# mavmap/mavmap

Measured on AMD Instinct MI355X. Metric: global-BA LM iterations/sec, higher is better.
Workload: dtype f64; 1 GPU; C3: 500 images / 200000 points / 2000000 obs global BA, PINHOLE+OPENCV, 2 shared cameras; images=500, points=200000, observations=2000000, parallelism=single GPU, options=max_iter 200, ftol 1e-6, gtol 1e-10, ptol 1e-8, Cauchy a=1, refine intrinsics

## Files before the change

include/mavba.h:

```cpp
#ifndef MAVBA_H_
#define MAVBA_H_

#include <stddef.h>
#include <stdint.h>

#ifdef __cplusplus
extern "C" {
#endif

#define MAVBA_VERSION 1

#define MAVBA_MODEL_PINHOLE 1
#define MAVBA_MODEL_OPENCV 2
#define MAVBA_MODEL_CATA 3
#define MAVBA_MAX_INTR 9

#define MAVBA_CONST_RVEC 1u
#define MAVBA_CONST_TX 2u
#define MAVBA_CONST_TY 4u
#define MAVBA_CONST_TZ 8u
#define MAVBA_CONST_POSE 15u

#define MAVBA_OK 0
#define MAVBA_ERR_INVALID_ARGUMENT (-1)
// ... 135 lines not shown
                        const int64_t* rot_image_ids, const double* rot_rvecs, int64_t n_rot,
                        const mavba_scene_options* scene_options, mavba_problem* problem, const int64_t** image_ids,
                        const int64_t** camera_ids, const int64_t** point_ids);

int mavba_scene_bundle_adjust(mavba_scene* s, const int64_t* free_ids, int64_t n_free, const int64_t* fixed_ids, int64_t n_fixed,
                              const int64_t* fixed_x_ids, int64_t n_fixed_x, const int64_t* gcp_ids, int64_t n_gcp,
                              const int64_t* rot_image_ids, const double* rot_rvecs, int64_t n_rot,
                              const mavba_scene_options* scene_options, const mavba_options* options, mavba_result* result,
                              double* final_cost_px, const int64_t** error_point_ids, const double** error_values,
                              int64_t* num_errors);

typedef struct mavba_session mavba_session;

int mavba_session_create(const mavba_problem* problem,
                         const mavba_options* options, mavba_session** out);
void mavba_session_destroy(mavba_session* s);

int mavba_session_reset(mavba_session* s);

int mavba_session_iterate(mavba_session* s, int32_t max_iters,
                          int32_t* iters_done, int32_t* termination);

int mavba_session_result(mavba_session* s, mavba_result* result);

int mavba_session_get_params(mavba_session* s, double* poses,
                             double* intrinsics, double* points);

int mavba_session_point_errors(mavba_session* s, double* point_error);

int mavba_session_set_params(mavba_session* s, const double* poses, const double* intrinsics, const double* points);

int mavba_session_restart(mavba_session* s);

int mavba_session_filter_points(mavba_session* s, double max_error, const uint8_t* keep, uint8_t* removed,
                                double* errors, int64_t* num_removed);

typedef int (*mavba_allreduce_fn)(void* ctx, void* device_ptr, int64_t count,
                                  int32_t op);
int mavba_session_set_allreduce(mavba_session* s, mavba_allreduce_fn fn,
                                void* ctx, int32_t rank, int32_t world_size);

int mavba_rccl_unique_id(void* out128);
int mavba_session_set_rccl(mavba_session* s, const void* unique_id128, int32_t rank, int32_t world_size);


int mavba_session_eval_jacobian(mavba_session* s, double* cost, double* r,
                                double* Jc, double* Jp, double* Jk);

int mavba_debug_inproc_comms(int32_t world, int32_t calls, int32_t abort_after, int64_t* out);

int mavba_debug_elimination_tree(int32_t num_images, int32_t num_cameras, int64_t npairs, const int32_t* pair_a,
                                 const int32_t* pair_b, int32_t max_depth, int32_t* node_of_image, int32_t* node_parent,
                                 int32_t cap);

int mavba_debug_radix_sort(int32_t n, const uint32_t* keys, int32_t key_bytes, int32_t* order_out, int32_t device);
int64_t mavba_debug_upload_batch(int32_t n, const int64_t* sizes, int64_t arena_bytes, int32_t device);
int mavba_debug_lm_decide(int32_t n, const double* cases, double* out_host, double* out_device, int32_t device);
int mavba_debug_chol_schedule(int32_t nb, int32_t num_nodes, const int32_t* node_begin, const int32_t* node_end, const int32_t* node_parent,
                              int64_t num_pairs, const int32_t* pair_row, const int32_t* pair_col, int32_t cus, double* out,
                              int32_t* tasks_out, int64_t tasks_cap, int64_t* num_tasks, int32_t* upd_out, int64_t upd_cap,
                              int64_t* num_upd, int32_t* chain_info_out);

int mavba_session_reduced_dim(mavba_session* s);
int mavba_session_reduced_system(mavba_session* s, double radius, double* S,
                                 double* v);

int mavba_session_linear_step(mavba_session* s, double radius, double* d_poses,
                              double* d_intr, double* d_points,
                              double* model_cost_change);

int mavba_session_time_jacobian(mavba_session* s, int32_t reps, float* ms_avg);
int mavba_session_set_profiling(mavba_session* s, int32_t on);
int mavba_session_time_front(mavba_session* s, double radius, int32_t reps, float* ms_avg);

typedef struct mavba_session_info {
  int64_t num_obs_kept;
  int32_t reduced_dim;
  int32_t padded_dim;
  int64_t schur_terms[3];
  int64_t schur_blocks;
  int64_t intr_entries;
  int64_t envelope_tiles;
  int64_t dense_tiles;
  double factor_flops;
  double dense_factor_flops;
  int32_t matrix_dim;
  int32_t nd_parts;
  int32_t chain_steps;
  int32_t num_clusters;
  int64_t clustered_points;
  int64_t cluster_partials;
  double cluster_flops;
  double chol_model_forward_us;
  int64_t reduced_store_bytes;
} mavba_session_info;
int mavba_session_get_info(mavba_session* s, mavba_session_info* out);

typedef struct mavba_kernel_stat {
  char name[48];
  int64_t launches;
  double total_ms;
} mavba_kernel_stat;
int mavba_session_kernel_stats(mavba_session* s, mavba_kernel_stat* out,
                               int32_t cap);

int mavba_dense_spd_solve(int32_t n, const double* A, const double* b,
// ... 7 lines not shown
```

mavmap_amd/__init__.py:

```python
from . import _abi
from .problem import BAProblem
from .api import (BundleAdjustmentOptions, MavbaError, Scene, Session, bundle_adjustment,
                  bundle_adjustment_filter_rebundle, pose_refinement, pose_refinement_batch, device_count, dense_spd_solve, rccl_unique_id, load, lib_path, radix_sort_order, elimination_tree, debug_upload_batch)
```

mavmap_amd/api.py:

```python
import ctypes as C
import os
from dataclasses import dataclass

import numpy as np

from . import _abi as A
from .problem import BAProblem

_LIB_PATH = os.path.join(os.path.dirname(os.path.abspath(__file__)), "lib", "libmavba.so")
_lib = None

EXPORTED_SYMBOLS = [
    "mavba_options_init", "mavba_last_error", "mavba_device_count", "mavba_solve", "mavba_pose_refine",
    "mavba_session_create", "mavba_session_destroy", "mavba_session_reset", "mavba_session_iterate",
    "mavba_session_result", "mavba_session_get_params", "mavba_session_point_errors",
    "mavba_session_set_allreduce", "mavba_session_eval_jacobian", "mavba_session_reduced_dim",
    "mavba_session_reduced_system", "mavba_session_linear_step", "mavba_session_time_jacobian", "mavba_session_time_front", "mavba_session_set_profiling",
    "mavba_session_kernel_stats", "mavba_session_get_info", "mavba_dense_spd_solve",
    "mavba_scene_create", "mavba_scene_destroy", "mavba_scene_set_camera", "mavba_scene_set_image", "mavba_scene_add_point2d",
    "mavba_scene_add_points2d", "mavba_scene_set_point3d", "mavba_scene_link", "mavba_scene_delete_point3d", "mavba_scene_get_image", "mavba_scene_get_point3d",
    "mavba_scene_get_camera", "mavba_scene_flatten", "mavba_scene_bundle_adjust",
    "mavba_rccl_unique_id", "mavba_session_set_rccl", "mavba_pose_refine_batch", "mavba_session_set_params", "mavba_session_restart", "mavba_session_filter_points", "mavba_solve_filter_solve",
    "mavba_debug_elimination_tree", "mavba_debug_radix_sort", "mavba_debug_lm_decide", "mavba_debug_chol_schedule",
    "mavba_debug_inproc_comms", "mavba_debug_upload_batch",
]

ALLREDUCE_FN = C.CFUNCTYPE(C.c_int, C.c_void_p, C.c_void_p, C.c_int64, C.c_int32)


class MavbaError(RuntimeError):
    def __init__(self, code, msg):
        super().__init__(f"mavba error {code}: {msg}")
        self.code = code


def lib_path():
    return _LIB_PATH


def load():
    global _lib
    if _lib is not None:
        return _lib
    if not os.path.exists(_LIB_PATH):
        raise MavbaError(A.ERR_NO_DEVICE, f"{_LIB_PATH} is missing: run `python -m mavmap_amd.build` "
                                          "(the HIP extension is mandatory, there is no CPU fallback)")
    L = C.CDLL(_LIB_PATH)
    dp, ip, bp = C.POINTER(C.c_double), C.POINTER(C.c_int32), C.POINTER(C.c_uint8)
    pp, op, rp = C.POINTER(A.CProblem), C.POINTER(A.COptions), C.POINTER(A.CResult)
    sp = C.c_void_p
    L.mavba_options_init.argtypes = [op]
    L.mavba_options_init.restype = None
    L.mavba_last_error.restype = C.c_char_p
    L.mavba_device_count.restype = C.c_int
    L.mavba_solve.argtypes = [pp, op, rp, dp]
    L.mavba_pose_refine.argtypes = [dp, dp, dp, C.c_int32, dp, dp, bp, C.c_int64, op, rp]
    L.mavba_session_create.argtypes = [pp, op, C.POINTER(sp)]
    L.mavba_session_destroy.argtypes = [sp]
    L.mavba_session_destroy.restype = None
    L.mavba_session_reset.argtypes = [sp]
    L.mavba_session_iterate.argtypes = [sp, C.c_int32, ip, ip]
    L.mavba_session_result.argtypes = [sp, rp]
    L.mavba_session_get_params.argtypes = [sp, dp, dp, dp]
    L.mavba_session_point_errors.argtypes = [sp, dp]
    L.mavba_session_set_allreduce.argtypes = [sp, ALLREDUCE_FN, C.c_void_p, C.c_int32, C.c_int32]
    L.mavba_session_eval_jacobian.argtypes = [sp, dp, dp, dp, dp, dp]
    L.mavba_session_reduced_dim.argtypes = [sp]
    L.mavba_session_reduced_system.argtypes = [sp, C.c_double, dp, dp]
    L.mavba_session_linear_step.argtypes = [sp, C.c_double, dp, dp, dp, dp]
    L.mavba_session_time_jacobian.argtypes = [sp, C.c_int32, C.POINTER(C.c_float)]
    L.mavba_session_time_front.argtypes = [sp, C.c_double, C.c_int32, C.POINTER(C.c_float)]
    L.mavba_session_set_profiling.argtypes = [sp, C.c_int32]
    L.mavba_session_kernel_stats.argtypes = [sp, C.POINTER(A.CKernelStat), C.c_int32]
    L.mavba_session_get_info.argtypes = [sp, C.POINTER(A.CSessionInfo)]
    L.mavba_dense_spd_solve.argtypes = [C.c_int32, dp, dp, dp, C.c_int32]
    i64p, i64 = C.POINTER(C.c_int64), C.c_int64
    sop = C.POINTER(A.CSceneOptions)
    L.mavba_scene_create.argtypes = [C.POINTER(sp)]
    L.mavba_scene_destroy.argtypes = [sp]
    L.mavba_scene_destroy.restype = None
    L.mavba_scene_set_camera.argtypes = [sp, i64, C.c_int32, dp]
    L.mavba_scene_set_image.argtypes = [sp, i64, i64, dp, dp]
    L.mavba_scene_add_point2d.argtypes = [sp, i64, i64, dp]
    L.mavba_scene_add_points2d.argtypes = [sp, i64, i64, i64p, dp, i64p]
    L.mavba_scene_set_point3d.argtypes = [sp, i64, dp]
    L.mavba_scene_link.argtypes = [sp, i64, i64]
    L.mavba_scene_delete_point3d.argtypes = [sp, i64]
    L.mavba_scene_get_image.argtypes = [sp, i64, dp, dp]
    L.mavba_scene_get_point3d.argtypes = [sp, i64, dp]
    L.mavba_scene_get_camera.argtypes = [sp, i64, ip, dp]
    lists = [i64p, i64, i64p, i64, i64p, i64, i64p, i64, i64p, dp, i64]
    L.mavba_scene_flatten.argtypes = [sp] + lists + [sop, pp, C.POINTER(i64p), C.POINTER(i64p), C.POINTER(i64p)]
    L.mavba_scene_bundle_adjust.argtypes = [sp] + lists + [sop, op, rp, dp, C.POINTER(i64p), C.POINTER(dp), i64p]
    L.mavba_rccl_unique_id.argtypes = [C.c_void_p]
    L.mavba_session_set_rccl.argtypes = [sp, C.c_void_p, C.c_int32, C.c_int32]
    L.mavba_pose_refine_batch.argtypes = [C.c_int32, C.POINTER(A.CPoseRefineItem), op, rp]
    L.mavba_session_set_params.argtypes = [sp, dp, dp, dp]
    L.mavba_session_restart.argtypes = [sp]
    L.mavba_session_filter_points.argtypes = [sp, C.c_double, bp, bp, dp, C.POINTER(C.c_int64)]
    L.mavba_solve_filter_solve.argtypes = [pp, op, C.c_double, bp, rp, rp, dp, bp, C.POINTER(C.c_int64)]
    L.mavba_debug_elimination_tree.argtypes = [C.c_int32, C.c_int32, C.c_int64, ip, ip, C.c_int32, ip, ip, C.c_int32]
    L.mavba_debug_radix_sort.argtypes = [C.c_int32, C.POINTER(C.c_uint32), C.c_int32, ip, C.c_int32]
    L.mavba_debug_lm_decide.argtypes = [C.c_int32, dp, dp, dp, C.c_int32]
    i32p, i64p = C.POINTER(C.c_int32), C.POINTER(C.c_int64)
    L.mavba_debug_chol_schedule.argtypes = [C.c_int32, C.c_int32, i32p, i32p, i32p, C.c_int64, i32p, i32p, C.c_int32, dp,
                                            i32p, C.c_int64, i64p, i32p, C.c_int64, i64p, i32p]
    for f in EXPORTED_SYMBOLS:
        if f not in ("mavba_options_init", "mavba_last_error", "mavba_session_destroy", "mavba_scene_destroy", "mavba_debug_upload_batch"):
            getattr(L, f).restype = C.c_int
    _lib = L
    return L


def _check(rc):
    if rc != A.OK:
        raise MavbaError(rc, load().mavba_last_error().decode(errors="replace"))


def device_count():
    return int(load().mavba_device_count())


def _d(a):
    return A.ptr(a, C.c_double)


@dataclass
class BundleAdjustmentOptions:
    max_num_iterations: int = 100
    function_tolerance: float = 1e-4
    gradient_tolerance: float = 1e-8
    update_point3D_errors: bool = False
    min_track_len: int = 2
    loss_scale_factor: float = 1.0
    constrain_rotation: bool = False
    constrain_rotation_weight: float = 0.0
    refine_camera_params: bool = False
    print_progress: bool = False
    print_summary: bool = True

    @staticmethod
    def global_ba():
        return BundleAdjustmentOptions(max_num_iterations=200, function_tolerance=1e-6,
                                       gradient_tolerance=1e-10, update_point3D_errors=True,
                                       refine_camera_params=True, print_summary=False)


def make_options(opts=None, **kw):
    o = A.COptions()
    load().mavba_options_init(C.byref(o))
    if isinstance(opts, BundleAdjustmentOptions):
        o.max_num_iterations = int(opts.max_num_iterations)
        o.function_tolerance = float(opts.function_tolerance)
        o.gradient_tolerance = float(opts.gradient_tolerance)
# ... 305 lines not shown

    def reduced_system(self, radius):
        n = load().mavba_session_reduced_dim(self._h)
        S, v = np.zeros((n, n)), np.zeros(n)
        _check(load().mavba_session_reduced_system(self._h, float(radius), _d(S), _d(v)))
        return S, v

    def linear_step(self, radius):
        p = self.problem
        dp, di, dx = np.zeros((p.num_images, 6)), np.zeros((p.num_cameras, 9)), np.zeros((p.num_points, 3))
        mcc = C.c_double()
        _check(load().mavba_session_linear_step(self._h, float(radius), _d(dp), _d(di), _d(dx), C.byref(mcc)))
        return dict(d_poses=dp, d_intr=di, d_points=dx, model_cost_change=mcc.value)

    def set_profiling(self, on):
        _check(load().mavba_session_set_profiling(self._h, 1 if on else 0))

    def time_front(self, radius=1e4, reps=20):
        ms = C.c_float(0)
        _check(load().mavba_session_time_front(self._h, float(radius), int(reps), C.byref(ms)))
        return ms.value

    def time_jacobian(self, reps=20):
        ms = C.c_float()
        _check(load().mavba_session_time_jacobian(self._h, int(reps), C.byref(ms)))
        return float(ms.value)

    def info(self):
        i = A.CSessionInfo()
        _check(load().mavba_session_get_info(self._h, C.byref(i)))
        d = {k: getattr(i, k) for k, _ in i._fields_ if k != "schur_terms"}
        d["schur_terms"] = list(i.schur_terms)
        return d

    def kernel_stats(self):
        buf = (A.CKernelStat * 64)()
        n = load().mavba_session_kernel_stats(self._h, buf, 64)
        return {buf[i].name.decode(): dict(launches=int(buf[i].launches), total_ms=float(buf[i].total_ms))
                for i in range(min(n, 64))}


def elimination_tree(num_images, num_cameras, pairs, max_depth=3):
    pairs = np.ascontiguousarray(pairs, dtype=np.int32).reshape(-1, 2)
    a, b = np.ascontiguousarray(pairs[:, 0]), np.ascontiguousarray(pairs[:, 1])
    node = np.zeros(max(num_images, 1), np.int32)
    parent = np.zeros(4096, np.int32)
    n = load().mavba_debug_elimination_tree(int(num_images), int(num_cameras), len(a), A.ptr(a, C.c_int32), A.ptr(b, C.c_int32),
                                           int(max_depth), A.ptr(node, C.c_int32), A.ptr(parent, C.c_int32), len(parent))
    if n < 0:
        _check(n)
    return node[:num_images], parent[:n]


def radix_sort_order(keys, key_bytes=4, device=-1):
    keys = np.ascontiguousarray(keys, dtype=np.uint32)
    out = np.zeros(len(keys), np.int32)
    _check(load().mavba_debug_radix_sort(len(keys), A.ptr(keys, C.c_uint32), int(key_bytes), A.ptr(out, C.c_int32), device))
    return out


def debug_upload_batch(sizes, arena_bytes=0, device=-1):
    sizes = np.ascontiguousarray(sizes, dtype=np.int64)
    f = load().mavba_debug_upload_batch
    f.restype = C.c_int64
    r = f(C.c_int32(len(sizes)), A.ptr(sizes, C.c_int64), C.c_int64(int(arena_bytes)), C.c_int32(device))
    if r < 0:
        raise MavbaError(A.ERR_HIP, load().mavba_last_error().decode(errors="replace"))
    return int(r)


def debug_lm_decide(cases, device=-1):
    cases = np.ascontiguousarray(cases, dtype=np.float64)
    n = cases.shape[0]
    assert cases.shape[1] == 24
    oh, od = np.zeros((n, 6)), np.zeros((n, 6))
    _check(load().mavba_debug_lm_decide(n, _d(cases), _d(oh), _d(od), device))
    return oh, od


def debug_chol_schedule(nb, nodes, pairs, cus=256):
    nodes = np.ascontiguousarray(nodes, dtype=np.int32).reshape(-1, 3)
    pairs = np.ascontiguousarray(pairs, dtype=np.int32).reshape(-1, 2)
    nbg, ne, npar = (np.ascontiguousarray(nodes[:, k]) for k in range(3))
    pr, pc = np.ascontiguousarray(pairs[:, 0]), np.ascontiguousarray(pairs[:, 1])
    i32 = lambda a: a.ctypes.data_as(C.POINTER(C.c_int32))
    out = np.zeros(8)
    nt, nu = C.c_int64(), C.c_int64()
    ci = np.zeros(nb, np.int32)
    L = load()
    _check(L.mavba_debug_chol_schedule(nb, len(nodes), i32(nbg), i32(ne), i32(npar), len(pairs), i32(pr), i32(pc), cus, _d(out),
                                       None, 0, C.byref(nt), None, 0, C.byref(nu), i32(ci)))
    tasks = np.zeros((max(nt.value, 1), 6), np.int32)
    upd = np.zeros(max(nu.value, 1), np.int32)
    _check(L.mavba_debug_chol_schedule(nb, len(nodes), i32(nbg), i32(ne), i32(npar), len(pairs), i32(pr), i32(pc), cus, _d(out),
                                       i32(tasks), nt.value, C.byref(nt), i32(upd), nu.value, C.byref(nu), i32(ci)))
    tl = [(int(t[0]), int(t[1]), int(t[2]), int(t[3]), [int(x) for x in upd[t[4]:t[5]]]) for t in tasks[:nt.value]]
    return dict(ok=bool(out[0]), model_forward_us=float(out[1]), launch_per_panel_us=float(out[2]), grid=int(out[3]),
                chain_wgs=int(out[4]), tiles=int(out[5]), updates=int(out[6]), nodes=int(out[7]), tasks=tl, chain_info=ci.tolist())


def rccl_unique_id():
    buf = C.create_string_buffer(128)
    _check(load().mavba_rccl_unique_id(buf))
    return buf.raw


# ... 6 lines not shown
```

mavmap_amd/build.py:

```python
import os
import shutil
import subprocess
import sys

ROOT = os.path.dirname(os.path.abspath(__file__))
CSRC = os.path.join(ROOT, "csrc")
LIBDIR = os.path.join(ROOT, "lib")
LIB = os.path.join(LIBDIR, "libmavba.so")
OBJDIR = os.path.join(LIBDIR, "obj")
SOURCES = ["kernels.hip", "schur_rows.hip", "dense_chol.hip", "pose_refine.hip", "host_util.hip", "session_build.hip", "session_lm.hip", "scene.hip", "multi_gpu.hip", "device_setup.hip", "api.hip"]
HEADERS = ["ba_math.h", "dev_reduce.h", "internal.h", "session.h", "lm_decide.h", "lm_bodies.h", "sweep_body.h", os.path.join("..", "..", "include", "mavba.h")]
FLAGS = ["--offload-arch=gfx950", "-O3", "-std=c++17", "-fPIC", "-ffp-contract=on", "-Wall",
         "-Wno-unused-result"]
FILE_FLAGS = {"dense_chol.hip": ["-mllvm", "-amdgpu-mfma-vgpr-form=1"]}


def _hipcc():
    for cand in (shutil.which("hipcc"), "/opt/rocm/bin/hipcc"):
        if cand and os.path.exists(cand):
            return cand
    raise RuntimeError("hipcc not found (ROCm toolchain required to build libmavba.so)")


STAMP = os.path.join(LIBDIR, "build_stamp.json")


def source_digest():
    import hashlib
    h = hashlib.sha256()
    for f in SOURCES + HEADERS:
        with open(os.path.normpath(os.path.join(CSRC, f)), "rb") as fh:
            h.update(f.encode() + b"\0" + fh.read())
    h.update(" ".join(FLAGS).encode())
    h.update(repr(sorted(FILE_FLAGS.items())).encode())
    return h.hexdigest()


def is_current():
    import json
    try:
        return os.path.exists(LIB) and json.load(open(STAMP))["digest"] == source_digest()
    except (OSError, ValueError, KeyError):
        return False


def _stale(target, deps):
    if not os.path.exists(target):
        return True
    t = os.path.getmtime(target)
    return any(os.path.getmtime(d) > t for d in deps if os.path.exists(d))


def build(force=False, verbose=False):
    os.makedirs(OBJDIR, exist_ok=True)
    hdrs = [os.path.normpath(os.path.join(CSRC, h)) for h in HEADERS]
    hipcc = _hipcc()
    objs = []
    for src in SOURCES:
        sp = os.path.join(CSRC, src)
        obj = os.path.join(OBJDIR, src.replace(".hip", ".o"))
        if force or _stale(obj, [sp] + hdrs):
            cmd = [hipcc] + FLAGS + FILE_FLAGS.get(src, []) + ["-c", sp, "-o", obj]
            if verbose:
                print(" ".join(cmd), file=sys.stderr)
            subprocess.check_call(cmd)
        objs.append(obj)
    if force or _stale(LIB, objs):
        cmd = [hipcc, "--offload-arch=gfx950", "-shared", "-fPIC", "-o", LIB] + objs
        if verbose:
            print(" ".join(cmd), file=sys.stderr)
        subprocess.check_call(cmd)
    if not is_current():
        import json
        with open(STAMP, "w") as fh:
            json.dump(dict(digest=source_digest()), fh)
    return LIB


if __name__ == "__main__":
    print(build(force="--force" in sys.argv, verbose=True))
```

mavmap_amd/csrc/api.hip:

```cpp
#include "session.h"
#include "lm_decide.h"

namespace mavba { thread_local std::string g_last_error; }

using namespace mavba;


#define MAVBA_TRY try {
namespace {
struct DeviceGuard {
  int prev = -1;
  explicit DeviceGuard(int dev) {
    if (hipGetDevice(&prev) != hipSuccess) { (void)hipGetLastError(); prev = -1; }
    if (prev != dev) HIP_OK(hipSetDevice(dev)); else prev = -1;
  }
  ~DeviceGuard() { if (prev >= 0) (void)hipSetDevice(prev); }
  DeviceGuard(const DeviceGuard&) = delete;
  DeviceGuard& operator=(const DeviceGuard&) = delete;
};
}
#define MAVBA_SESSION_TRY(s)                                                    \
  try {                                                                         \
    if (!(s)) throw Failure(MAVBA_ERR_INVALID_ARGUMENT, "null session");        \
    DeviceGuard device_guard_((s)->device);
// ... 269 lines not shown
  MAVBA_SESSION_TRY(s)
  s->evaluate();
  if (cost) *cost = s->cost + s->fixed_cost;
  s->ensure_planes();
  launch_jacobian_sweep(s->st, s->sweep_args(s->d_camrec.p, s->d_intr.p, s->d_points.p));
  const size_t S = s->Nstride, N = s->N;
  auto pull = [&](const double* dev, int planes, std::vector<double>& h) {
    h.resize((size_t)planes * S);
    s->download(h.data(), dev, h.size() * 8);
  };
  std::vector<double> hR, hJp, hJc, hJk;
  pull(s->d_R.p, 2, hR); pull(s->d_Jp.p, 6, hJp); pull(s->d_Jc.p, 12, hJc); pull(s->d_Jk.p, 2 * s->KMAX, hJk);
  s->sync();
  s->ensure_perm_host();
  const size_t NO = (size_t)s->NO_all;
  if (r) std::memset(r, 0, NO * 2 * 8);
  if (Jc) std::memset(Jc, 0, NO * 12 * 8);
  if (Jp) std::memset(Jp, 0, NO * 6 * 8);
  if (Jk) std::memset(Jk, 0, NO * 18 * 8);
  for (size_t a = 0; a < N; ++a) {
    const size_t o = (size_t)s->perm[a];
    if (r) for (int e = 0; e < 2; ++e) r[o * 2 + e] = hR[e * S + a];
    if (Jp) for (int e = 0; e < 6; ++e) Jp[o * 6 + e] = hJp[e * S + a];
    if (Jc) for (int e = 0; e < 12; ++e) Jc[o * 12 + e] = hJc[e * S + a];
    if (Jk)
      for (int row = 0; row < 2; ++row)
        for (int k = 0; k < s->KMAX; ++k) Jk[o * 18 + row * 9 + k] = hJk[(size_t)(row * s->KMAX + k) * S + a];
  }
  return MAVBA_OK;
  MAVBA_CATCH
}

int mavba_session_reduced_dim(mavba_session* s) { return s ? s->n_full : 0; }

int mavba_debug_elimination_tree(int32_t NI, int32_t NC, int64_t npairs, const int32_t* pair_a, const int32_t* pair_b, int32_t max_depth,
                                 int32_t* node_of_image, int32_t* node_parent, int32_t cap) {
  MAVBA_TRY
  if (NI < 0 || NC < 0 || npairs < 0 || (npairs > 0 && (!pair_a || !pair_b)) || !node_of_image || !node_parent)
    throw Failure(MAVBA_ERR_INVALID_ARGUMENT, "bad argument");
  std::vector<std::vector<int>> lower(NI);
  for (int64_t k = 0; k < npairs; ++k) {
    const int a = pair_a[k], b = pair_b[k];
    if (a < 0 || a >= NI || b < 0 || b >= NI) throw Failure(MAVBA_ERR_BAD_INDEX, "image pair out of range");
    if (a != b) lower[std::max(a, b)].push_back(std::min(a, b));
  }
  const std::vector<ElimNode> tn = elimination_tree(NI, NC, lower, -1, max_depth);
  if ((int)tn.size() > cap) throw Failure(MAVBA_ERR_INVALID_ARGUMENT, "node_parent too small");
  for (int i = 0; i < NI; ++i) node_of_image[i] = -1;
  for (size_t t = 0; t < tn.size(); ++t) {
    node_parent[t] = tn[t].parent;
    for (int i : tn[t].imgs) node_of_image[i] = (int)t;
  }
  return (int)tn.size();
  MAVBA_CATCH
}

int mavba_session_reduced_system(mavba_session* s, double radius, double* Sout, double* vout) {
  MAVBA_SESSION_TRY(s)
  if (!s->evaluated) s->evaluate();
  s->assemble(radius);
  const int n = s->n_full, m = s->n_mat, nbt = m / 64;
  std::vector<double> store(s->chol_struct.store_doubles());
  s->download(store.data(), s->d_M.p, store.size() * 8);
  s->sync();
  std::vector<double> h((size_t)(m + 1) * m, 0.0);
  const std::vector<int>& slot = s->chol_struct.tile_slot;
  for (int tr = 0; tr <= nbt; ++tr)
    for (int tc = 0; tc < nbt; ++tc) {
      const int sl = slot[(size_t)tr * nbt + tc];
      if (sl < 0) continue;
      const double* T = &store[(size_t)sl << 12];
      const int rows = tr < nbt ? 64 : 1;
      for (int r = 0; r < rows; ++r) std::memcpy(&h[(size_t)(64 * tr + r) * m + 64 * tc], T + 64 * r, 64 * 8);
    }
  std::vector<int> var_col(n, 0);
  for (int t = 0; t < m; ++t) if (s->h_col_var[t] >= 0) var_col[s->h_col_var[t]] = t;
  if (Sout)
    for (int r = 0; r < n; ++r)
      for (int c = 0; c < n; ++c) {
        const int a = std::max(var_col[r], var_col[c]), b = std::min(var_col[r], var_col[c]);
        Sout[(size_t)r * n + c] = h[(size_t)a * m + b];
      }
  if (vout)
    for (int r = 0; r < n; ++r) vout[r] = h[(size_t)m * m + var_col[r]];
  return MAVBA_OK;
  MAVBA_CATCH
}

int mavba_session_linear_step(mavba_session* s, double radius, double* d_poses, double* d_intr, double* d_points,
                              double* model_cost_change) {
  MAVBA_SESSION_TRY(s)
  if (!s->evaluated) s->evaluate();
  double h[SC_COUNT];
  s->linear_step(radius, h);
  if (model_cost_change) *model_cost_change = h[SC_MODEL_CHANGE];
  if (d_poses && s->NI) s->download(d_poses, s->d_delta_cam.p, (size_t)s->NI * 48);
  if (d_intr && s->NC) s->download(d_intr, s->d_delta_cam.p + 6 * (size_t)s->NI, (size_t)s->NC * 72);
  std::vector<double> hdp;
  if (d_points && s->NP) { hdp.resize((size_t)s->NP * 3); s->download(hdp.data(), s->d_delta_pts.p, (size_t)s->NP * 24); }
  s->sync();
  if (d_points) s->to_caller_points(hdp.data(), d_points, 3);
  if (h[SC_FAIL] != 0.0 || h[SC_FAIL_FRONT] != 0.0) throw Failure(MAVBA_ERR_INVALID_ARGUMENT, "linear solve failed (matrix not positive definite)");
  return MAVBA_OK;
  MAVBA_CATCH
}

// ... 417 lines not shown
```

mavmap_amd/csrc/ba_math.h:

```cpp
#ifndef MAVBA_BA_MATH_H_
#define MAVBA_BA_MATH_H_

#include <math.h>

#if defined(__HIPCC__)
#include <hip/hip_runtime.h>
#define MAVBA_HD __host__ __device__ __forceinline__
#else
#define MAVBA_HD inline
#endif

#define MAVBA_M_PINHOLE 1
#define MAVBA_M_OPENCV 2
#define MAVBA_M_CATA 3

namespace mavba {

MAVBA_HD void rot_coeffs(double th2, double& a, double& b, double& c) {
  if (th2 > 1e-6) {
    const double th = sqrt(th2);
    const double s = sin(th), co = cos(th);
    a = s / th;
    b = (1.0 - co) / th2;
    c = (th - s) / (th2 * th);
// ... 167 lines not shown
  double dz0 = 0.0, dz1 = 0.0, dz2 = 1.0;
  if (model == MAVBA_M_CATA) {
    if (nrm > 0.0) {
      const double s = cam[8] / nrm;
      dz0 = s * Xc[0]; dz1 = s * Xc[1]; dz2 = 1.0 + s * Xc[2];
    }
    const double dun = -un * nrm * iz, dvn = -vn * nrm * iz;
    su += (D0 * dun + D1 * dvn) * dk[8];
    sv += (D2 * dun + D3 * dvn) * dk[8];
  }
  const double n0 = iz - un * iz * dz0, n1 = -un * iz * dz1, n2 = -un * iz * dz2;
  const double n3 = -vn * iz * dz0, n4 = iz - vn * iz * dz1, n5 = -vn * iz * dz2;
  A[0] = fx * (D0 * n0 + D1 * n3); A[1] = fx * (D0 * n1 + D1 * n4); A[2] = fx * (D0 * n2 + D1 * n5);
  A[3] = fy * (D2 * n0 + D3 * n3); A[4] = fy * (D2 * n1 + D3 * n4); A[5] = fy * (D2 * n2 + D3 * n5);
  tk0 = ud * dk[0] + dk[2] + fx * su;
  tk1 = vd * dk[1] + dk[3] + fy * sv;
}

MAVBA_HD void obs_residual(int model, const double* rec, const double* cam, const double* X,
                           double uo, double vo, double* r) {
  double Xr[3], Xc[3], u, v;
  transform_point(rec, X, Xr, Xc);
  project<false>(model, cam, Xc, u, v, nullptr, nullptr);
  r[0] = u - uo; r[1] = v - vo;
}

MAVBA_HD void obs_jacobian(int model, const double* rec, const double* cam, const double* X,
                           double uo, double vo, double* r, double* Jc, double* Jp, double* Jk) {
  double Xr[3], Xc[3], u, v, A[6];
  transform_point(rec, X, Xr, Xc);
  project<true>(model, cam, Xc, u, v, A, Jk);
  r[0] = u - uo; r[1] = v - vo;
  const double a = rec[6], b = rec[7], c = rec[8];
#pragma unroll
  for (int i = 0; i < 2; ++i) {
    const double* Ai = &A[3 * i];
    double m1[3], m2[3];
    cross3(Ai, rec, m1);
    cross3(m1, rec, m2);
    Jp[3 * i + 0] = Ai[0] + a * m1[0] + b * m2[0];
    Jp[3 * i + 1] = Ai[1] + a * m1[1] + b * m2[1];
    Jp[3 * i + 2] = Ai[2] + a * m1[2] + b * m2[2];
    double n[3];
    cross3(Ai, Xr, n);
    cross3(n, rec, m1);
    cross3(m1, rec, m2);
    Jc[6 * i + 0] = -(n[0] + b * m1[0] + c * m2[0]);
    Jc[6 * i + 1] = -(n[1] + b * m1[1] + c * m2[1]);
    Jc[6 * i + 2] = -(n[2] + b * m1[2] + c * m2[2]);
    Jc[6 * i + 3] = Ai[0]; Jc[6 * i + 4] = Ai[1]; Jc[6 * i + 5] = Ai[2];
  }
}

MAVBA_HD void obs_backsub_term(int model, const double* rec, const double* cam, const double* X, double uo, double vo,
                               const double* dc, const double* dk, double* r, double* t) {
  double Xr[3], Xc[3], u, v, A[6], tk0, tk1;
  transform_point(rec, X, Xr, Xc);
  project_dk(model, cam, Xc, dk, u, v, A, tk0, tk1);
  r[0] = u - uo; r[1] = v - vo;
  const double a = rec[6], b = rec[7], c = rec[8];
  double m1[3], m2[3], om[3], dX[3];
  cross3(rec, dc, m1);
  cross3(rec, m1, m2);
  om[0] = dc[0] + b * m1[0] + c * m2[0]; om[1] = dc[1] + b * m1[1] + c * m2[1]; om[2] = dc[2] + b * m1[2] + c * m2[2];
  cross3(om, Xr, dX);
  dX[0] += dc[3]; dX[1] += dc[4]; dX[2] += dc[5];
  const double tau0 = A[0] * dX[0] + A[1] * dX[1] + A[2] * dX[2] + tk0;
  const double tau1 = A[3] * dX[0] + A[4] * dX[1] + A[5] * dX[2] + tk1;
  const double q[3] = {A[0] * tau0 + A[3] * tau1, A[1] * tau0 + A[4] * tau1, A[2] * tau0 + A[5] * tau1};
  cross3(rec, q, m1);
  cross3(rec, m1, m2);
  t[0] = q[0] - a * m1[0] + b * m2[0]; t[1] = q[1] - a * m1[1] + b * m2[1]; t[2] = q[2] - a * m1[2] + b * m2[2];
}

MAVBA_HD void cauchy_weight(double s, double b, double inv_b, double& w, double& half_rho) {
  const double sum = 1.0 + s * inv_b;
  half_rho = 0.5 * b * log_obs(sum);
  w = rsqrt_obs(sum);
}

MAVBA_HD void rot_matrix_colmajor(const double* w, double* R) {
  double a, b, c;
  const double th2 = w[0] * w[0] + w[1] * w[1] + w[2] * w[2];
  rot_coeffs(th2, a, b, c);
  const double x = w[0], y = w[1], z = w[2];
  R[0] = 1.0 + b * (x * x - th2); R[3] = -a * z + b * x * y;      R[6] = a * y + b * x * z;
  R[1] = a * z + b * x * y;       R[4] = 1.0 + b * (y * y - th2); R[7] = -a * x + b * y * z;
  R[2] = -a * y + b * x * z;      R[5] = a * x + b * y * z;       R[8] = 1.0 + b * (z * z - th2);
}

MAVBA_HD void rot_prior_eval(const double* w, const double* R0, double weight, double& res,
                             double* jac) {
  const double x = w[0], y = w[1], z = w[2];
  const double th2 = x * x + y * y + z * z;
  double a, b, c;
  rot_coeffs(th2, a, b, c);
  double a1, b1;
  if (th2 > 1e-6) {
    const double th = sqrt(th2), s = sin(th), co = cos(th);
    a1 = (th * co - s) / (th2 * th);
    b1 = (th * s - 2.0 * (1.0 - co)) / (th2 * th2);
  } else {
    a1 = -1.0 / 3.0 + th2 * (1.0 / 30.0 - th2 / 840.0);
    b1 = -1.0 / 12.0 + th2 * (1.0 / 180.0 - th2 / 6720.0);
  }
  const double W[9] = {0, -z, y, z, 0, -x, -y, x, 0};
  const double W2[9] = {x * x - th2, x * y, x * z, x * y, y * y - th2, y * z, x * z, y * z, z * z - th2};
  double R[9];
#pragma unroll
  for (int i = 0; i < 9; ++i) R[i] = ((i % 4 == 0) ? 1.0 : 0.0) + a * W[i] + b * W2[i];
  const int ia[9] = {0, 3, 6, 1, 4, 7, 2, 6, 8};
  double d[9], acc = 0.0;
#pragma unroll
  for (int k = 0; k < 9; ++k) {
    const int cm = ia[k];
    d[k] = R[(cm % 3) * 3 + cm / 3] - R0[k];
    acc += d[k] * d[k];
  }
  const double nrm = sqrt(acc);
  res = weight * nrm;
#pragma unroll
  for (int m = 0; m < 3; ++m) {
    double E[9] = {0, 0, 0, 0, 0, 0, 0, 0, 0};
    if (m == 0) { E[5] = -1; E[7] = 1; }
    if (m == 1) { E[2] = 1; E[6] = -1; }
// ... 55 lines not shown
```

mavmap_amd/csrc/dense_chol.hip:

```cpp
#include "internal.h"
#include "lm_bodies.h"
#include <algorithm>
#include <cstdio>
#include <cstdlib>
#include <iterator>
#include <mutex>
#include <type_traits>

namespace mavba {

namespace {
constexpr int NB = 64;
constexpr int GLD = 66;

typedef double d4 __attribute__((ext_vector_type(4)));

[[maybe_unused]] __device__ __forceinline__ double rsqrt_nr(double d) {
  double y = __builtin_amdgcn_rsq(d);
  const double hd = 0.5 * d;
  y = y * (1.5 - hd * y * y);
  y = y * (1.5 - hd * y * y);
  return y;
}

// ... 99 lines not shown
  const d4 U = __builtin_amdgcn_mfma_f64_16x16x4f64(xa, ba, zero, 0, 0, 0);
  const d4 Xn = __builtin_amdgcn_mfma_f64_16x16x4f64(xa, xacc[B], zero, 0, 0, 0);
  __builtin_amdgcn_sched_barrier(0);
  const double u = li >= c0 + lk ? U[0] : 0.0;
  acc = __builtin_amdgcn_mfma_f64_16x16x4f64(-u, u, acc, 0, 0, 0);
  xacc = __builtin_amdgcn_mfma_f64_16x16x4f64(-u, Xn[0], xacc, 0, 0, 0);
  xfin[B] = Xn[0];
}
__device__ __forceinline__ bool potrf_inv16_b4(d4& acc, d4& xacc, int lane) {
  bool ok = true;
  const int li = lane & 15, lk = lane >> 4;
  d4 xfin = (d4){0.0, 0.0, 0.0, 0.0};
#pragma unroll
  for (int r = 0; r < 4; ++r) xacc[r] = (lk + 4 * r == li) ? 1.0 : 0.0;
  const Pivot4Masks mk = pivot4_masks(lane);
  potrf_inv16_block4<0>(acc, xacc, xfin, lane, ok, mk);
  potrf_inv16_block4<1>(acc, xacc, xfin, lane, ok, mk);
  potrf_inv16_block4<2>(acc, xacc, xfin, lane, ok, mk);
  potrf_inv16_block4<3>(acc, xacc, xfin, lane, ok, mk);
  xacc = xfin;
  const double last = readlane_d(xfin[3], 63);
  return last == last;
}

__device__ __forceinline__ d4 gemm16(const double* A, int lda, const double* B, int ldb, bool transB,
                                     double sign, d4 acc, int lane) {
  const int li = lane & 15, lk = lane >> 4;
#pragma unroll
  for (int kk = 0; kk < 16; kk += 4) {
    const double av = sign * A[li * lda + kk + lk];
    const double bv = transB ? B[li * ldb + kk + lk] : B[(kk + lk) * ldb + li];
    acc = __builtin_amdgcn_mfma_f64_16x16x4f64(av, bv, acc, 0, 0, 0);
  }
  return acc;
}
__device__ __forceinline__ d4 load_d16(const double* C, int ldc, int lane) {
  const int li = lane & 15, lk = lane >> 4;
  d4 v;
#pragma unroll
  for (int r = 0; r < 4; ++r) v[r] = C[(lk + 4 * r) * ldc + li];
  return v;
}
__device__ __forceinline__ void store_d16(double* C, int ldc, d4 v, int lane) {
  const int li = lane & 15, lk = lane >> 4;
#pragma unroll
  for (int r = 0; r < 4; ++r) C[(lk + 4 * r) * ldc + li] = v[r];
}

constexpr bool kPivot4 = true;
constexpr int kFuseBelow = 24;
constexpr int kFuseTasks = 256;
constexpr int kMaxBacksolveGroups = 2048;

__device__ __forceinline__ void wave_lds_sync() {
  __builtin_amdgcn_fence(__ATOMIC_RELEASE, "wavefront");
  __builtin_amdgcn_wave_barrier();
  __builtin_amdgcn_fence(__ATOMIC_ACQUIRE, "wavefront");
}

struct NoPhaseHook { __device__ __forceinline__ void operator()(int) const {} };
struct NoMark { __device__ __forceinline__ void operator()(int) const {} };
struct NoPhase0 { __device__ __forceinline__ void operator()(int) const {} };
template <class Hook = NoPhaseHook, class Mark = NoMark, class Phase0 = NoPhase0>
__device__ __forceinline__ bool tile_potrf_inv_la(double* T, double* Ti, int tid, Hook hook = Hook(), Mark mark = Mark(),
                                                  Phase0 phase0 = Phase0()) {
  const int wv = tid >> 6, lane = tid & 63;
  const d4 zero = (d4){0.0, 0.0, 0.0, 0.0};
  auto Tb = [&](int i, int j) { return T + (16 * i) * GLD + 16 * j; };
  auto Xb = [&](int i, int j) { return Ti + (16 * i) * GLD + 16 * j; };
  auto Lb = [&](int i, int j) { return Ti + (16 * j) * GLD + 16 * i; };
  auto panel = [&](const double* B, const double* Dinv, double* dst) {
    d4 a = gemm16(B, GLD, Dinv, GLD, true, 1.0, zero, lane);
    store_d16(dst, GLD, a, lane);
  };
  auto downdate = [&](double* C, const double* Pa, const double* Pb) {
    d4 a = load_d16(C, GLD, lane);
    a = gemm16(Pa, GLD, Pb, GLD, true, -1.0, a, lane);
    store_d16(C, GLD, a, lane);
  };
  auto chain = [&](double* C, const double* P, int c) -> bool {
    d4 a = load_d16(C, GLD, lane), x;
    if (P) a = gemm16(P, GLD, P, GLD, true, -1.0, a, lane);
    mark(4 * c + 1);
    {
      const int li = lane & 15, lk = lane >> 4;
      bool ident = true;
#pragma unroll
      for (int r = 0; r < 4; ++r) ident = ident && a[r] == ((lk + 4 * r == li) ? 1.0 : 0.0);
      if (__builtin_amdgcn_ballot_w64(!ident) == 0) {
        if (c == 0) phase0(1);
        store_d16(Xb(c, c), GLD, a, lane);
        mark(4 * c + 2);
        return true;
      }
    }
    const bool ok = kPivot4 ? potrf_inv16_b4(a, x, lane) : potrf_inv16(a, x, lane);
    mark(4 * c + 2);
    if (c == 0) phase0(1);
    store_d16(Xb(c, c), GLD, x, lane);
    return ok;
  };
  bool ok = true;
  if (wv == 0) { phase0(0); ok = chain(Tb(0, 0), nullptr, 0); }
  else phase0(2);
  __syncthreads();
  hook(0);
  if (wv != 0) phase0(3);
  if (wv == 0) {
    mark(3);
    panel(Tb(1, 0), Xb(0, 0), Lb(1, 0));
    wave_lds_sync();
// ... 1966 lines not shown
      for (int i = 0; i < NB; i += 2) { s0 = __builtin_fma(Li[i * GLD + lane], in[i], s0); s1 = __builtin_fma(Li[(i + 1) * GLD + lane], in[i + 1], s1); }
      out[lane] = s0 + s1;
    }
  };
  lower_mv(I0, vv, zz);
  if (nb > 1) {
    d4 acc[2][2];
    mfma_quadrant_nt(P, I0, wr, wc, lane, acc);
    load_tile_or_zero(M, sl.s11, W, tid);
    __syncthreads();
    quadrant_to_lds(P, wr, wc, lane, acc);
    __syncthreads();
    d4 upd[2][2], cur[2][2];
    mfma_quadrant_nt(P, P, wr, wc, lane, upd);
    quadrant_from_lds(W, wr, wc, lane, cur);
    quadrant_sub(cur, upd);
    if (wv == 0) {
      double s0 = 0.0, s1 = 0.0;
#pragma unroll 8
      for (int j = 0; j < NB; j += 2) { s0 = __builtin_fma(P[lane * GLD + j], zz[j], s0); s1 = __builtin_fma(P[lane * GLD + j + 1], zz[j + 1], s1); }
      xx[NB + lane] = vv[NB + lane] - (s0 + s1);
    }
    __syncthreads();
    quadrant_to_lds(W, wr, wc, lane, cur);
    __syncthreads();
    ok = tile_factor_inverse(W, I1, tid) && ok;
    __syncthreads();
    lower_mv(I1, xx + NB, zz + NB);
    __syncthreads();
    lower_tmv(I1, zz + NB, xx + NB);
    __syncthreads();
    if (wv == 0) {
      double s0 = 0.0, s1 = 0.0;
#pragma unroll 8
      for (int i = 0; i < NB; i += 2) { s0 = __builtin_fma(P[i * GLD + lane], xx[NB + i], s0); s1 = __builtin_fma(P[(i + 1) * GLD + lane], xx[NB + i + 1], s1); }
      zz[lane] -= s0 + s1;
    }
  }
  __syncthreads();
  lower_tmv(I0, zz, xx);
  __syncthreads();
  if (tid == 0 && !ok) atomicAdd(fail, 1.0);
  for (int c = tid; c < nb_all * NB; c += 256) {
    const double x = c < nb * NB ? xx[c] : 0.0;
    y[c] = x;
    if (scatter) { const int t = scatter[c]; if (t >= 0) y_nat[t] = x; }
  }
  if (UPD) {
    __shared__ double s_red[4];
    __syncthreads();
    const int groups = (U.NI + kUpdImagesPerGroup - 1) / kUpdImagesPerGroup;
    for (int vb = 0; vb < (groups > 0 ? groups : 1); ++vb) {
      update_cameras_body(vb, U.NI, U.NC, U.cam_part, U.radius, U.dmin, U.dmax, y_nat, U.scale_cam, U.img_rec, U.cam_rec, U.poses, U.intr,
                          U.cand_poses, U.cand_intr, U.delta_cam, U.partial3, U.cand_camrec, s_red);
      __syncthreads();
    }
  }
}

static bool chol_small_path() {
  static const bool on = [] { const char* e = std::getenv("MAVBA_CHOL_SMALL"); return !e || std::atoi(e) != 0; }();
  return on;
}
bool dense_spd_solve_is_small(int n_pad, const CholStructure& cs) {
  const int nb = n_pad / NB;
  const int nb_active = cs.active_tiles > 0 ? std::min(cs.active_tiles, nb) : nb;
  return nb_active <= 2 && chol_small_path();
}
bool dense_spd_solve_device(hipStream_t st, double* M, int n_pad, double* y, double* fail,
                            double* diag_ws, double* L, const CholStructure& cs,
                            const int* y_scatter, double* y_nat, bool allow_persistent, hipEvent_t after_factor,
                            const CamUpdateArgs* upd) {
  const int nb = n_pad / NB;
  const int* slot = cs.d_tile_slot;
  double* inv = diag_ws;
  const int nb_active = cs.active_tiles > 0 ? std::min(cs.active_tiles, nb) : nb;
  if (dense_spd_solve_is_small(n_pad, cs)) {
    const bool with_update = upd != nullptr && y_scatter != nullptr && y_nat != nullptr;
    auto hs = [&](int i, int k) { return i <= nb && k < nb ? cs.tile_slot[(size_t)i * nb + k] : -1; };
    const SmallSlots sl{hs(0, 0), nb > 1 ? hs(1, 0) : -1, nb > 1 ? hs(1, 1) : -1, hs(nb, 0), nb > 1 ? hs(nb, 1) : -1};
    if (with_update)
      hipLaunchKernelGGL(k_chol_small<true>, dim3(1), dim3(256), 0, st, M, sl, nb, nb_active, fail, y, y_scatter, y_nat, *upd);
    else
      hipLaunchKernelGGL(k_chol_small<false>, dim3(1), dim3(256), 0, st, M, sl, nb, nb_active, fail, y, y_scatter, y_nat, CamUpdateArgs{});
    if (after_factor) (void)hipEventRecord(after_factor, st);
    return with_update;
  }
  const unsigned epoch = ++cs.epoch;
  if (allow_persistent && cs.persist_ok) {
    CholPersistArgs A;
    A.M = M; A.L = L; A.inv = inv; A.pre = cs.d_pre; A.nb = nb;
    A.tasks = cs.d_tasks; A.wg_begin = cs.d_wg_begin; A.upd = cs.d_upd; A.tile_id = cs.d_tile_id; A.chain_info = cs.d_chain_info;
    A.lflag = cs.d_pflags; A.dflag = cs.d_pflags + cs.persist_tiles; A.pflag = A.dflag + nb; A.abort_flag = A.pflag + 2 * nb;
    A.epoch = epoch; A.fail = fail; A.trace = cs.d_trace;
    static const int drop = [] { const char* e = std::getenv("MAVBA_CHOL_TEST_DROP_WG"); return e ? std::atoi(e) : -1; }();
    A.drop_wg = drop;
    {
      static std::mutex chain_m;
      static hipEvent_t last[64] = {};
      static hipStream_t only_stream[64] = {};
      static bool chained[64] = {};
      int dev = 0;
      (void)hipGetDevice(&dev);
      const bool tracked = dev >= 0 && dev < 64;
      std::lock_guard<std::mutex> g(chain_m);
      if (tracked && !chained[dev]) {
        if (!only_stream[dev]) only_stream[dev] = st;
// ... 63 lines not shown
```

mavmap_amd/csrc/dev_reduce.h:

```cpp
#ifndef MAVBA_DEV_REDUCE_H_
#define MAVBA_DEV_REDUCE_H_
#include <hip/hip_runtime.h>

namespace mavba {

__device__ __forceinline__ double wave_sum(double v) {
#define MAVBA_ROR_ADD(N)                                                                                   \
  {                                                                                                        \
    const int lo = __builtin_amdgcn_update_dpp(0, __double2loint(v), 0x120 | (N), 0xf, 0xf, false);        \
    const int hi = __builtin_amdgcn_update_dpp(0, __double2hiint(v), 0x120 | (N), 0xf, 0xf, false);        \
    v += __hiloint2double(hi, lo);                                                                         \
  }
  MAVBA_ROR_ADD(8) MAVBA_ROR_ADD(4) MAVBA_ROR_ADD(2) MAVBA_ROR_ADD(1)
#undef MAVBA_ROR_ADD
  const int lo = __double2loint(v), hi = __double2hiint(v);
  const double r0 = __hiloint2double(__builtin_amdgcn_readlane(hi, 0), __builtin_amdgcn_readlane(lo, 0));
  const double r1 = __hiloint2double(__builtin_amdgcn_readlane(hi, 16), __builtin_amdgcn_readlane(lo, 16));
  const double r2 = __hiloint2double(__builtin_amdgcn_readlane(hi, 32), __builtin_amdgcn_readlane(lo, 32));
  const double r3 = __hiloint2double(__builtin_amdgcn_readlane(hi, 48), __builtin_amdgcn_readlane(lo, 48));
  return (r0 + r1) + (r2 + r3);
}
__device__ __forceinline__ double wave_max(double v) {
#pragma unroll
  for (int off = 32; off > 0; off >>= 1) v = fmax(v, __shfl_down(v, off, 64));
  return v;
}

__device__ __forceinline__ double dev_rsqrt(double d) {
  const double y = __builtin_amdgcn_rsq(d);
  const double h = __builtin_fma(-(d * y), y, 1.0);
  return __builtin_fma(y * h, __builtin_fma(0.375, h, 0.5), y);
}
__device__ __forceinline__ bool chol3_inv_fast(const double* C, double* Gi) {
  const double r0 = dev_rsqrt(C[0]);
  const double l10 = C[1] * r0, l20 = C[2] * r0;
  const double d1 = __builtin_fma(-l10, l10, C[3]);
  const double r1 = dev_rsqrt(d1);
  const double l21 = __builtin_fma(-l20, l10, C[4]) * r1;
  const double d2 = __builtin_fma(-l21, l21, __builtin_fma(-l20, l20, C[5]));
  const double r2 = dev_rsqrt(d2);
  Gi[0] = r0;
  Gi[1] = -(l10 * r0) * r1;
  Gi[2] = r1;
  Gi[4] = -(l21 * r1) * r2;
  Gi[3] = -__builtin_fma(l21, Gi[1], l20 * r0) * r2;
  Gi[5] = r2;
  return (C[0] > 0.0) && (d1 > 0.0) && (d2 > 0.0);
}

__device__ __forceinline__ double block_sum_256(double v, double* scratch) {
  v = wave_sum(v);
  const int lane = threadIdx.x & 63, wv = threadIdx.x >> 6;
  __syncthreads();
  if (lane == 0) scratch[wv] = v;
  __syncthreads();
  return (scratch[0] + scratch[1]) + (scratch[2] + scratch[3]);
}
// ... 14 lines not shown
```

mavmap_amd/csrc/internal.h:

```cpp
#ifndef MAVBA_INTERNAL_H_
#define MAVBA_INTERNAL_H_

#include <hip/hip_runtime.h>
#include <stdint.h>

#include <utility>
#include <vector>
#include <functional>

namespace mavba {

constexpr int kPoseRec = 24;
constexpr int kIntrRec = 36;

constexpr int kImgRec = 81;
constexpr int kCamRec = 54;
constexpr int kSweepAcc = 135;

struct SweepChunk { int image; int begin; int end; };

enum { BLK_PP = 0, BLK_IP = 1, BLK_II = 2 };

struct SchurBlock {
  int kind;
// ... 155 lines not shown
                      const double* poses, double* res, double* jac, double* cost_partial, const LmSpec& spec = lm_spec_off());

void launch_scales(hipStream_t st, int NI, int NC, int NP, int NPs, int jacobi,
                   const unsigned char* pose_free, const unsigned char* intr_free,
                   const unsigned char* pt_free, const double* img_rec, const double* cam_rec,
                   const double* Cu, double* scale_cam, double* scale_pt);

constexpr int kStateNormsCamBlocks = 64;
void launch_state_norms(hipStream_t st, int NI, int NC, int NP, int NPs, bool cam_part,
                        const unsigned char* pose_free, const unsigned char* intr_free,
                        const unsigned char* pt_free, const double* poses, const double* intr,
                        const double* points, const double* img_rec, const double* cam_rec,
                        const double* gu, double* partial , int* grid_out, const LmSpec& spec = lm_spec_off());


void launch_entries_pose(hipStream_t st, int N, int Nstride, int NPs, const int* obs_img,
                         const int* obs_pt, const unsigned char* pt_free, const double* Jc,
                         const double* Jp, const double* scale_cam, const double* scale_pt,
                         double* Gi, double* h, double* Epose);
void launch_factor_entries_pose(hipStream_t st, int N, int Nstride, int NPs, const int* obs_img, const int* obs_pt,
                                const unsigned char* pt_free, const double* Jc, const double* Jp, const double* scale_cam,
                                const double* scale_pt, double* Gi, double* h, double* Epose, const int* pt_start,
                                const double* Cu, const double* gu, double radius, double dmin, double dmax, double* fail);
void launch_entries_intr(hipStream_t st, int Q, int NI, int NPs, const int* q_pt, const int* q_cam,
                         const double* Wk, const double* scale_cam, const double* scale_pt,
                         const double* Gi, const double* h, double* Eintr);

void launch_schur_chunks(hipStream_t st, int kind, int num_chunks, const SchurChunk* chunks,
                         const int2* terms, const double* Epose, const double* Eintr,
                         double* partial);
int schur_partial_stride(int kind);
void launch_schur_rows(hipStream_t st, const FrontArgs& a, int kmax_intr, bool generic, int num_clusters,
                       const SchurRowsCluster* clusters, const int* tab, const int* cl_lists, const unsigned short* obs_meta,
                       const unsigned long long* lanemap, const unsigned* emit_map, double* part_pp, double* part_ip, double* part_ii,
                       const struct CamSweepArgs* with_sweep = nullptr );
void rows_emit_map(int ni, int nc, int flags, std::vector<unsigned>& pass0, std::vector<unsigned>& pass1);
constexpr unsigned long long kRowsLanesIdentity = 0xFEDCBA9876543210ull;
void launch_schur_clusters(hipStream_t st, ClusterShape shape, int num_clusters, const SchurCluster* clusters, const int* tab,
                           const int* pt_start, const int* q_start, const unsigned short* obs_meta,
                           const unsigned short* q_meta, const unsigned char* pt_clustered, const double* Epose,
                           const double* Eintr, const double* h, int NPs, double* part_pp, double* part_ip,
                           double* part_ii);
void launch_schur_finalize(hipStream_t st, int num_blocks, const SchurBlock* blocks,
                           const double* part_pp, const double* part_ip, const double* part_ii,
                           int NI, int NC, const int* slot, int nb, bool add_base, double radius, double dmin,
                           double dmax, const int* img_cam, const double* img_rec,
                           const double* cam_rec, const double* scale_cam, const int* off_img, const int* off_cam,
                           double* S);
void launch_tiles_copy(hipStream_t st, int num_tiles, const int* tiles, const int* slot, int nb, double* M, double* buf, bool to_buf);
void launch_fix_diag(hipStream_t st, int n_mat, const int* slot, bool add_one, const int* col_var,
                     const double* scale_cam, double* S);

int backsub_points_grid(int NP);
void launch_backsub_points_jvp(hipStream_t st, int NP, int NPs, int NI, double radius, double dmin, double dmax,
                               const SweepArgs& a, const int* pt_start, const double* delta_cam,
                               const unsigned char* pt_free, const double* Gi, const double* h, const double* Cu,
                               const double* gu, const double* scale_pt, double* cand_points, double* delta_points,
                               double* partial , const double* cand_camrec = nullptr, const double* cand_intr = nullptr,
                               double* cost_partial = nullptr);
int update_cameras_groups(int NI);
void launch_update_cameras(hipStream_t st, int NI, int NC, bool cam_part, double radius, double dmin,
                           double dmax, const double* y, const double* scale_cam,
                           const double* img_rec, const double* cam_rec, const double* poses,
                           const double* intr, double* cand_poses, double* cand_intr,
                           double* delta_cam, double* partial3 , double* cand_camrec );

void launch_reduce_cols(hipStream_t st, const double* partial, int rows, int cols, int stride,
                        unsigned max_mask, double* out, bool accumulate);

struct ReduceTask { const double* src; int rows, stride, is_max; const double* src2; int rows2; double* out; };
struct ReduceTasks { ReduceTask t[6]; };
void launch_reduce_tasks(hipStream_t st, const ReduceTasks& tasks, int n, const LmSpec& spec = lm_spec_off());
constexpr int kLmPubDoubles = SC_COUNT + 8;
void launch_lm_snapshot(hipStream_t st, const LmSpec& spec, double* dec, double* host_pub, double seq, double* fail_slots );
void launch_lm_decide_cases(hipStream_t st, int n, const double* in, double* out);
void launch_lm_tail(hipStream_t st, const ReduceTasks& tasks, int n, const LmSpec& spec, double* dec, double* host_pub, double seq, double* fail_slots);
void state_norms_grid(int NI, int NC, int NP, int* gp, int* gc);
struct EvalSmallArgs {
  int NI, NC, NP, NPs, with_cams, cam_part, gp, gc, num_tasks;
  int first_group = 0;
  const int* img_chunk_start; const double* cam_partial; const int* prior_start; const double* prior_res; const double* prior_jac;
  const int* cam_img_start; const int* cam_imgs; double* img_rec; double* cam_rec; double* img_intr_tmp;
  const unsigned char* pose_free; const unsigned char* intr_free; const unsigned char* pt_free;
  const double* poses; const double* intr; const double* points; const double* gu; double* norm_partial;
  ReduceTasks T; LmSpec spec;
  PartialRide ride;
};
void launch_eval_small(hipStream_t st, const EvalSmallArgs& a);
void launch_eval_head_tail(hipStream_t st, const EvalSmallArgs& a);
bool eval_head_tail_fits(int gc);

void launch_points_to_caller(hipStream_t st, int NP, int width, const int* orig, const double* in, double* out);
void launch_point_errors(hipStream_t st, int NP, const int* pt_start, const double* rnorm,
                         const int* pt_count, double* perr);

hipError_t device_alloc(void** p, size_t bytes);
void device_free(void* p);
hipError_t copy_h2d_staged(void* dst, const void* src, size_t bytes, hipStream_t st);
hipError_t copy_d2h_staged_sync(void* dst, const void* src, size_t bytes, hipStream_t st);
void release_staged(hipStream_t st);
bool upload_batch_begin(hipStream_t st);
hipError_t upload_batch_end(bool emit);
hipError_t zero_async(void* p, size_t bytes, hipStream_t st);
void upload_batch_debug_arena(size_t bytes);
int host_threads();
void host_run(int T, const std::function<void(int)>& body);

struct CholFront {
  int k;
  int na;
  int act_off;
  int factor_next;
  int sh_begin;
  long long sh_off;
};
struct CholStep { int kind, front_off, nf, nf0, max_na, merge_begin, init_off, tasks; };
struct CholMerge { int sh_begin; long long sh_off; };
struct CholNode { int begin, end, parent; };
// ... 8 lines not shown
  std::vector<CholMerge> merges;
  std::vector<CholStep> steps;
  std::vector<int> init_tiles;
  int num_leaf_init = 0;
  int chain_steps = 0;
  int num_fronts_max = 0;
  long long envelope_tiles = 0;
  double factor_flops = 0.0;
  size_t shadow_doubles = 0;
  int* d_ints = nullptr;
  int *d_rows = nullptr, *d_seg_of_tile = nullptr, *d_seg_first = nullptr, *d_init = nullptr;
  unsigned* d_flags = nullptr;
  CholFront* d_fronts = nullptr;
  CholMerge* d_merges = nullptr;
  mutable double* d_shadow = nullptr;
  std::vector<int> tile_slot;
  int* d_tile_slot = nullptr;
  long long num_tiles = 0;
  size_t store_doubles() const { return (size_t)std::max<long long>(num_tiles, 1) * 4096; }
  int active_tiles = 0;
  bool persist_ok = false;
  double predicted_forward_us = 0.0;
  int persist_grid = 0;
  int persist_chain_wgs = 0;
  long long persist_tiles = 0;
  long long persist_updates = 0;
  CholTask* d_tasks = nullptr;
  int* d_pints = nullptr;
  int *d_wg_begin = nullptr, *d_upd = nullptr, *d_tile_id = nullptr, *d_chain_info = nullptr;
  unsigned* d_pflags = nullptr;
  double* d_pre = nullptr;
  unsigned long long* d_trace = nullptr;
  std::vector<CholTask> h_tasks;
  std::vector<int> h_wg_begin, h_upd, h_chain_info;
  bool host_only = false;
  int host_only_cus = 256;
  double lpp_estimate_us = 0.0;
  mutable unsigned epoch = 0;
  CholStructure() {}
  CholStructure(const CholStructure&) = delete;
  CholStructure& operator=(const CholStructure&) = delete;
  ~CholStructure();
  void release();
  hipError_t build(int nb, const std::vector<std::pair<int, int>>& tile_pairs, const std::vector<CholNode>& tree,
                   hipStream_t st);
  hipError_t build_dense(int nb);
  hipError_t build_persistent(const std::vector<std::vector<int>>& col_rows, const std::vector<int>& col_step,
                              const std::vector<int>& height, hipStream_t st);
};
struct CamUpdateArgs {
  int NI, NC, cam_part; double radius, dmin, dmax;
  const double* scale_cam; const double* img_rec; const double* cam_rec; const double* poses; const double* intr;
  double* cand_poses; double* cand_intr; double* delta_cam; double* partial3; double* cand_camrec;
};
bool dense_spd_solve_is_small(int n_pad, const CholStructure& cs);
bool dense_spd_solve_device(hipStream_t st, double* M, int n_pad, double* y, double* fail,
                            double* diag_ws, double* L, const CholStructure& cs,
                            const int* y_scatter = nullptr, double* y_nat = nullptr, bool allow_persistent = true,
                            hipEvent_t after_factor = nullptr ,
                            const CamUpdateArgs* upd = nullptr);

}
#endif
```

mavmap_amd/csrc/kernels.hip:

```cpp
#include "internal.h"
#include <cstdlib>
#include <type_traits>
#include "ba_math.h"
#include "dev_reduce.h"
#include "lm_decide.h"
#include "lm_bodies.h"
#include "sweep_body.h"

namespace mavba {

__global__ void k_cam_prepare(int NI, const double* __restrict__ poses, double* __restrict__ camrec) {
  const int i = blockIdx.x * blockDim.x + threadIdx.x;
  if (i >= NI) return;
  double rec[9];
  cam_prepare(poses + 6 * i, rec);
#pragma unroll
  for (int k = 0; k < 9; ++k) camrec[9 * i + k] = rec[k];
}
void launch_cam_prepare(hipStream_t st, int NI, const double* poses, double* camrec) {
  if (NI <= 0) return;
  hipLaunchKernelGGL(k_cam_prepare, dim3((NI + 127) / 128), dim3(128), 0, st, NI, poses, camrec);
}

constexpr int kSweepObsPerBlock = 512;
// ... 1451 lines not shown
        const double g = B.kind == BLK_PP ? img_rec[(size_t)B.row_ent * kImgRec + 21 + r]
                                          : cam_rec[(size_t)B.row_ent * kCamRec + 45 + r];
        base = scale_cam[gr] * g;
      }
      const int C = prow0 + r;
      S[((size_t)slot[nb * nb + (C >> 6)] << 12) + (C & 63)] = base - s;
    }
  };
  for (int idx = lane; idx < PS; idx += 64) apply(idx, strided_sum16(part, PS, idx, B.chunk_begin, B.chunk_end));
}
void launch_schur_finalize(hipStream_t st, int num_blocks, const SchurBlock* blocks,
                           const double* part_pp, const double* part_ip, const double* part_ii,
                           int NI, int NC, const int* slot, int nb, bool add_base, double radius, double dmin,
                           double dmax, const int* img_cam, const double* img_rec,
                           const double* cam_rec, const double* scale_cam, const int* off_img, const int* off_cam,
                           double* S) {
  if (num_blocks <= 0) return;
  hipLaunchKernelGGL(k_schur_finalize, dim3((num_blocks + 3) / 4), dim3(256), 0, st, num_blocks, blocks, part_pp,
                     part_ip, part_ii, NI, NC, slot, nb, add_base ? 1 : 0, radius, dmin, dmax, img_cam, img_rec, cam_rec,
                     scale_cam, off_img, off_cam, S);
}
__global__ void __launch_bounds__(256) k_tiles_copy(int num_tiles, const int* __restrict__ tiles, const int* __restrict__ slot, int nb,
                                                    double* __restrict__ M, double* __restrict__ buf, int to_buf) {
  const int t = blockIdx.x;
  if (t < num_tiles) {
    double2* a = reinterpret_cast<double2*>(M + ((size_t)tiles[t] << 12));
    double2* b = reinterpret_cast<double2*>(buf + ((size_t)t << 12));
    for (int e = threadIdx.x; e < 2048; e += 256) { if (to_buf) b[e] = a[e]; else a[e] = b[e]; }
  } else {
    double* rhs = buf + ((size_t)num_tiles << 12);
    for (int c = (t - num_tiles) * 256 + threadIdx.x; c < nb * 64; c += (gridDim.x - num_tiles) * 256) {
      double* a = M + ((size_t)slot[nb * nb + (c >> 6)] << 12) + (c & 63);
      if (to_buf) rhs[c] = *a; else *a = rhs[c];
    }
  }
}
void launch_tiles_copy(hipStream_t st, int num_tiles, const int* tiles, const int* slot, int nb, double* M, double* buf, bool to_buf) {
  const int extra = std::max(1, std::min(16, (nb * 64 + 1023) / 1024));
  hipLaunchKernelGGL(k_tiles_copy, dim3(num_tiles + extra), dim3(256), 0, st, num_tiles, tiles, slot, nb, M, buf, to_buf ? 1 : 0);
}

__global__ void k_fix_diag(int n_mat, const int* __restrict__ slot, int add_one, const int* __restrict__ col_var,
                           const double* __restrict__ scale_cam, double* __restrict__ S) {
  const int t = blockIdx.x * blockDim.x + threadIdx.x;
  if (t >= n_mat) return;
  const int j = col_var[t];
  if (j < 0 || scale_cam[j] == 0.0) S[((size_t)slot[(t >> 6) * (n_mat >> 6) + (t >> 6)] << 12) + (t & 63) * 65] = add_one ? 1.0 : 0.0;
}
void launch_fix_diag(hipStream_t st, int n_mat, const int* slot, bool add_one, const int* col_var, const double* scale_cam, double* S) {
  hipLaunchKernelGGL(k_fix_diag, dim3((n_mat + 255) / 256), dim3(256), 0, st, n_mat, slot, add_one ? 1 : 0, col_var, scale_cam, S);
}

constexpr int kBsCamsLds = 16;
__global__ void __launch_bounds__(256) k_backsub_points_packed(
    int NP, int NPs, int NI, int NC, int N, int ppb, int nblocks, double radius, double dmin, double dmax, double loss_b, double loss_inv_b,
    const int* __restrict__ pt_start, const int* __restrict__ obs_img, const int* __restrict__ obs_pt,
    const double2* __restrict__ uv, const int* __restrict__ img_cam, const int* __restrict__ cam_model,
    const double* __restrict__ camrec, const double* __restrict__ intr, const double* __restrict__ delta_cam,
    const unsigned char* __restrict__ pt_free, const double* __restrict__ Gi, const double* __restrict__ h,
    const double* __restrict__ Cu, const double* __restrict__ gu, const double* __restrict__ scale_pt,
    const double* __restrict__ points, double* __restrict__ cand_points, double* __restrict__ delta_points,
    double* __restrict__ partial, const double* __restrict__ cand_camrec, const double* __restrict__ cand_intr,
    const unsigned char* __restrict__ pt_active, double* __restrict__ cost_partial) {
  __shared__ double s_t[3][256];
  __shared__ double s_new[3][128];
  __shared__ double s_red[4];
  __shared__ double s_kin[kBsCamsLds][9], s_dk[kBsCamsLds][9];
  __shared__ int s_model[kBsCamsLds];
  const int tid = threadIdx.x;
  const bool cams_lds = NC <= kBsCamsLds;
  double a_step = 0.0, a_model = 0.0, a_x2 = 0.0, a_cost = 0.0;
  const int G = (int)gridDim.x;
  struct Obs { int pt, im; double2 m; };
  auto load_obs = [&](int o) {
    Obs r{0, 0, make_double2(0.0, 0.0)};
    if (N <= 0) return r;
    const int oc = min(o, N - 1);
    r.pt = obs_pt[oc]; r.im = obs_img[oc]; r.m = uv[oc];
    return r;
  };
  auto obs_term = [&](const Obs& q, bool valid, double (&t)[3]) {
    t[0] = t[1] = t[2] = 0.0;
    if (!valid || !pt_free[q.pt]) return;
    const int cam = img_cam[q.im];
    const double X[3] = {points[3 * (size_t)q.pt], points[3 * (size_t)q.pt + 1], points[3 * (size_t)q.pt + 2]};
    double rec[9], kin[9], dc[6], dk[9];
#pragma unroll
    for (int k = 0; k < 9; ++k) rec[k] = camrec[9 * q.im + k];
#pragma unroll
    for (int k = 0; k < 6; ++k) dc[k] = delta_cam[6 * q.im + k];
    int model;
    if (cams_lds) {
      model = s_model[cam];
#pragma unroll
      for (int k = 0; k < 9; ++k) { kin[k] = s_kin[cam][k]; dk[k] = s_dk[cam][k]; }
    } else {
      model = cam_model[cam];
#pragma unroll
      for (int k = 0; k < 9; ++k) { kin[k] = intr[9 * cam + k]; dk[k] = delta_cam[6 * NI + 9 * cam + k]; }
    }
    double r[2], tt[3];
#ifndef MAVBA_BS_SKIP
#define MAVBA_BS_SKIP 0
#endif
    if (MAVBA_BS_SKIP & 1) { r[0] = rec[0] + kin[0] + dc[0] + dk[0]; r[1] = X[0] + q.m.x; tt[0] = rec[3]; tt[1] = X[1]; tt[2] = q.m.y; }
    else
    obs_backsub_term(model, rec, kin, X, q.m.x, q.m.y, dc, dk, r, tt);
    double w, half_rho;
    cauchy_weight(r[0] * r[0] + r[1] * r[1], loss_b, loss_inv_b, w, half_rho);
    const double w2 = w * w;
    t[0] = w2 * tt[0]; t[1] = w2 * tt[1]; t[2] = w2 * tt[2];
  };
  int o0 = 0, o1 = 0, o0n = 0, o1n = 0;
  Obs cur{0, 0, make_double2(0.0, 0.0)};
  if ((int)blockIdx.x < nblocks) {
    const int b0 = (int)blockIdx.x;
    o0 = pt_start[b0 * ppb]; o1 = pt_start[min(b0 * ppb + ppb, NP)];
    if (b0 + G < nblocks) { o0n = pt_start[(b0 + G) * ppb]; o1n = pt_start[min((b0 + G) * ppb + ppb, NP)]; }
    cur = load_obs(o0 + tid);
  }
  if (cams_lds) {
    for (int e = tid; e < 9 * NC; e += 256) { s_kin[e / 9][e % 9] = intr[e]; s_dk[e / 9][e % 9] = delta_cam[6 * NI + e]; }
    for (int c = tid; c < NC; c += 256) s_model[c] = cam_model[c];
    __syncthreads();
  }
  for (int blk = blockIdx.x; blk < nblocks; blk += G) {
    const int p0 = blk * ppb, p1 = min(p0 + ppb, NP);
    const int p = p0 + tid;
    const bool owner = p < p1;
    int o0nn = 0, o1nn = 0;
    Obs nxt = cur;
    if (blk + G < nblocks) {
      nxt = load_obs(o0n + tid);
      if (blk + 2 * G < nblocks) { o0nn = pt_start[(blk + 2 * G) * ppb]; o1nn = pt_start[min((blk + 2 * G) * ppb + ppb, NP)]; }
    }
    int mb = 0, me = 0;
    bool fr = false;
    double G[6] = {0, 0, 0, 0, 0, 0}, sp[3] = {0, 0, 0}, hh[3] = {0, 0, 0}, cu[3] = {0, 0, 0}, gg[3] = {0, 0, 0}, Xo[3] = {0, 0, 0};
    if (owner) {
      mb = pt_start[p]; me = pt_start[p + 1];
      fr = pt_free[p] != 0;
#pragma unroll
      for (int k = 0; k < 3; ++k) Xo[k] = points[3 * (size_t)p + k];
      if (fr) {
        const int dg[3] = {0, 3, 5};
#pragma unroll
        for (int k = 0; k < 6; ++k) G[k] = Gi[k * NPs + p];
#pragma unroll
        for (int k = 0; k < 3; ++k) { sp[k] = scale_pt[k * NPs + p]; hh[k] = h[k * NPs + p]; cu[k] = Cu[dg[k] * NPs + p]; gg[k] = gu[k * NPs + p]; }
      }
    }
    double T[3] = {0.0, 0.0, 0.0};
    for (int base = o0; base < o1; base += 256) {
      const int o = base + tid;
      const Obs q = base == o0 ? cur : load_obs(o);
      double t[3];
      obs_term(q, o < o1, t);
      s_t[0][tid] = t[0]; s_t[1][tid] = t[1]; s_t[2][tid] = t[2];
      __syncthreads();
      if (owner) {
        const int b = max(mb, base), e = (MAVBA_BS_SKIP & 2) ? min(me, max(mb, base) + 1) : min(me, base + 256);
        for (int i = b; i < e; ++i) { T[0] += s_t[0][i - base]; T[1] += s_t[1][i - base]; T[2] += s_t[2][i - base]; }
      }
      __syncthreads();
    }
    if (owner) {
      double d[3] = {0, 0, 0};
      if (fr) {
        const double q0 = -sp[0] * T[0], q1 = -sp[1] * T[1], q2 = -sp[2] * T[2];
        const double z[3] = {q0 * G[0], q0 * G[1] + q1 * G[2], q0 * G[3] + q1 * G[4] + q2 * G[5]};
        const double tt[3] = {hh[0] - z[0], hh[1] - z[1], hh[2] - z[2]};
        double yp[3];
        git_mul(G, tt, yp);
#pragma unroll
        for (int k = 0; k < 3; ++k) {
          const double s = sp[k];
          const double D2 = clampd(s * s * cu[k], dmin, dmax) / radius;
          const double gs = s * gg[k];
          a_model += 0.5 * yp[k] * (gs + D2 * yp[k]);
          d[k] = -yp[k] * s;
          a_step += d[k] * d[k];
        }
      }
#pragma unroll
      for (int k = 0; k < 3; ++k) {
        const double xn = Xo[k] + d[k];
        cand_points[3 * (size_t)p + k] = xn;
        delta_points[3 * (size_t)p + k] = d[k];
        if (fr) a_x2 += xn * xn;
        if (cost_partial) s_new[k][tid] = xn;
      }
    }
    if (cost_partial) {
      __syncthreads();
      for (int base = o0; base < o1; base += 256) {
        const int o = base + tid;
        if (o < o1) {
          const int pt = obs_pt[o], im = obs_img[o];
          const double2 m = uv[o];
          const int cam = img_cam[im];
          double rec[9], kin[9], r[2];
#pragma unroll
          for (int k = 0; k < 9; ++k) rec[k] = cand_camrec[9 * im + k];
#pragma unroll
          for (int k = 0; k < 9; ++k) kin[k] = cand_intr[9 * cam + k];
          const double Xn[3] = {s_new[0][pt - p0], s_new[1][pt - p0], s_new[2][pt - p0]};
          obs_residual(cam_model[cam], rec, kin, Xn, m.x, m.y, r);
          double w, half_rho;
          cauchy_weight(r[0] * r[0] + r[1] * r[1], loss_b, loss_inv_b, w, half_rho);
          if (pt_active && !pt_active[pt]) half_rho = 0.0;
          a_cost += half_rho;
        }
      }
      __syncthreads();
    }
    o0 = o0n; o1 = o1n; o0n = o0nn; o1n = o1nn; cur = nxt;
  }
  const double s0 = block_sum_256(a_step, s_red);
  const double s1 = block_sum_256(a_model, s_red);
  const double s2 = block_sum_256(a_x2, s_red);
  if (threadIdx.x == 0) { partial[3 * blockIdx.x] = s0; partial[3 * blockIdx.x + 1] = s1; partial[3 * blockIdx.x + 2] = s2; }
  if (cost_partial) {
    const double s3 = block_sum_256(a_cost, s_red);
    if (threadIdx.x == 0) cost_partial[blockIdx.x] = s3;
  }
}
int backsub_points_grid(int NP) {
  int gp = (NP + 15) / 16;
  if (gp > 1024) gp = 1024;
  return gp < 1 ? 1 : gp;
}
void launch_backsub_points_jvp(hipStream_t st, int NP, int NPs, int NI, double radius, double dmin, double dmax,
                               const SweepArgs& a, const int* pt_start, const double* delta_cam,
                               const unsigned char* pt_free, const double* Gi, const double* h, const double* Cu,
                               const double* gu, const double* scale_pt, double* cand_points, double* delta_points,
                               double* partial, const double* cand_camrec, const double* cand_intr, double* cost_partial) {
  const int gp = backsub_points_grid(NP);
  const double track = NP > 0 ? (double)a.N / NP : 1.0;
  const int ppb = std::max(1, std::min(128, (int)(224.0 / std::max(track, 1.0))));
  const int nblocks = (NP + ppb - 1) / ppb;
  hipLaunchKernelGGL(k_backsub_points_packed, dim3(gp), dim3(256), 0, st, NP, NPs, NI, a.NC, a.N, ppb, nblocks, radius, dmin, dmax, a.loss_b,
                     a.loss_inv_b, pt_start, a.obs_img, a.obs_pt, a.uv, a.img_cam, a.cam_model, a.camrec, a.intr, delta_cam, pt_free,
                     Gi, h, Cu, gu, scale_pt, a.points, cand_points, delta_points, partial, cand_camrec, cand_intr, a.pt_active,
                     cost_partial);
}

int update_cameras_groups(int NI) { return std::max(1, (NI + kUpdImagesPerGroup - 1) / kUpdImagesPerGroup); }
__global__ void __launch_bounds__(256) k_update_cameras(
    int NI, int NC, int cam_part, double radius, double dmin, double dmax, const double* __restrict__ y,
    const double* __restrict__ scale_cam, const double* __restrict__ img_rec, const double* __restrict__ cam_rec,
    const double* __restrict__ poses, const double* __restrict__ intr, double* cand_poses,
    double* __restrict__ cand_intr, double* __restrict__ delta_cam, double* __restrict__ partial3,
    double* __restrict__ cand_camrec) {
  __shared__ double s_red[4];
  update_cameras_body(blockIdx.x, NI, NC, cam_part, radius, dmin, dmax, y, scale_cam, img_rec, cam_rec, poses, intr, cand_poses, cand_intr,
                      delta_cam, partial3, cand_camrec, s_red);
}
void launch_update_cameras(hipStream_t st, int NI, int NC, bool cam_part, double radius, double dmin,
                           double dmax, const double* y, const double* scale_cam,
                           const double* img_rec, const double* cam_rec, const double* poses,
                           const double* intr, double* cand_poses, double* cand_intr,
                           double* delta_cam, double* partial3, double* cand_camrec) {
  hipLaunchKernelGGL(k_update_cameras, dim3(update_cameras_groups(NI)), dim3(256), 0, st, NI, NC, cam_part ? 1 : 0, radius, dmin,
                     dmax, y, scale_cam, img_rec, cam_rec, poses, intr, cand_poses, cand_intr, delta_cam, partial3, cand_camrec);
}

__global__ void __launch_bounds__(256) k_reduce_cols(const double* __restrict__ partial, int rows, int cols,
                                                     int stride, unsigned max_mask, double* __restrict__ out,
                                                     int accumulate) {
  __shared__ double s_red[4];
  for (int c = 0; c < cols; ++c) {
    const bool mx = (max_mask >> c) & 1u;
    double v = 0.0;
    for (int r = threadIdx.x; r < rows; r += 256) {
      const double x = partial[(size_t)r * stride + c];
      v = mx ? fmax(v, x) : v + x;
    }
    const double t = mx ? block_max_256(v, s_red) : block_sum_256(v, s_red);
    if (threadIdx.x == 0) {
      if (accumulate) out[c] = mx ? fmax(out[c], t) : out[c] + t;
      else out[c] = t;
    }
    __syncthreads();
  }
}
void launch_reduce_cols(hipStream_t st, const double* partial, int rows, int cols, int stride,
                        unsigned max_mask, double* out, bool accumulate) {
  hipLaunchKernelGGL(k_reduce_cols, dim3(1), dim3(256), 0, st, partial, rows, cols, stride, max_mask, out, accumulate ? 1 : 0);
}

__global__ void __launch_bounds__(256) k_reduce_tasks(ReduceTasks T, LmSpec spec) {
  __shared__ double s_red[4];
  if (!lm_spec_go(spec, nullptr)) return;
  reduce_task_body(T.t[blockIdx.x], s_red);
}
__global__ void __launch_bounds__(64) k_lm_snapshot(LmSpec spec, double* dec, double* host_pub, double seq, double* fail_slots) {
  lm_snapshot_body(threadIdx.x, spec, dec, host_pub, seq, fail_slots);
}
__global__ void __launch_bounds__(1024) k_lm_tail(ReduceTasks T, int n, LmSpec spec, double* dec, double* host_pub, double seq, double* fail_slots) {
  __shared__ double s_t[4][2][4];
  reduce_tasks_grouped(T, n, s_t);
  if (threadIdx.x < 64) lm_snapshot_body(threadIdx.x, spec, dec, host_pub, seq, fail_slots);
}
constexpr int kEvalSmallMaxGroups = 40;
__global__ void __launch_bounds__(1024) k_eval_small(EvalSmallArgs a) {
  __shared__ double s_part[16][64];
  __shared__ double s_w[kEvalSmallMaxGroups][2][4];
  __shared__ double s_t[4][2][4];
  if (!lm_spec_go(a.spec, nullptr)) return;
  const int tid = threadIdx.x, g = tid >> 8, lt = tid & 255, wv = (tid >> 6) & 3, lane = tid & 63;
  for (int q = tid; q < a.NI * kSweepAcc; q += 1024)
    camera_reduce_img_elem(q / kSweepAcc, q % kSweepAcc, a.img_chunk_start, a.cam_partial, a.prior_start, a.prior_res, a.prior_jac, a.img_rec,
                           a.img_intr_tmp);
  __syncthreads();
  if (a.with_cams) {
    for (int c = 0; c < a.NC; ++c) {
      if (lane < kCamRec) s_part[tid >> 6][lane] = camera_reduce_cam_part(c, tid >> 6, lane, a.cam_img_start, a.cam_imgs, a.img_intr_tmp);
// ... 146 lines not shown
```

mavmap_amd/csrc/lm_bodies.h:

```cpp
#ifndef MAVBA_LM_BODIES_H_
#define MAVBA_LM_BODIES_H_
#include "internal.h"
#include "ba_math.h"
#include "dev_reduce.h"
#include "lm_decide.h"

namespace mavba {

__device__ __forceinline__ void camera_reduce_img_elem(int i, int e, const int* img_chunk_start, const double* partial,
                                                        const int* prior_start, const double* prior_res, const double* prior_jac,
                                                        double* img_rec, double* img_intr_tmp) {
  const int c0 = img_chunk_start[i], c1 = img_chunk_start[i + 1];
  double s = 0.0;
  int c = c0;
  for (; c + 4 <= c1; c += 4) {
    const double x0 = partial[(size_t)c * kSweepAcc + e], x1 = partial[(size_t)(c + 1) * kSweepAcc + e];
    const double x2 = partial[(size_t)(c + 2) * kSweepAcc + e], x3 = partial[(size_t)(c + 3) * kSweepAcc + e];
    s += x0; s += x1; s += x2; s += x3;
  }
  for (; c < c1; ++c) s += partial[(size_t)c * kSweepAcc + e];
  if (e < 27 && prior_start) {
    for (int q = prior_start[i]; q < prior_start[i + 1]; ++q) {
      const double* j = prior_jac + 3 * q;
      if (e < 21) {
// ... 68 lines not shown
  const double s = block_sum_256(x2, s_red);
  if (threadIdx.x == 0) { partial[2 * vb] = m; partial[2 * vb + 1] = s; }
}

__device__ __forceinline__ double group4_sum(const double* w) { return (w[0] + w[1]) + (w[2] + w[3]); }
__device__ __forceinline__ double group4_max(const double* w) { return fmax(fmax(w[0], w[1]), fmax(w[2], w[3])); }

__device__ __forceinline__ void reduce_task_body(const ReduceTask& t, double* s_red) {
  double v = 0.0;
  for (int r = threadIdx.x; r < t.rows; r += 256) {
    const double x = t.src[(size_t)r * t.stride];
    v = t.is_max ? fmax(v, x) : v + x;
  }
  double total = t.is_max ? block_max_256(v, s_red) : block_sum_256(v, s_red);
  if (t.rows2 > 0) {
    __syncthreads();
    double w = 0.0;
    for (int r = threadIdx.x; r < t.rows2; r += 256) w += t.src2[r];
    total += block_sum_256(w, s_red);
  }
  if (threadIdx.x == 0) *t.out = total;
}

__device__ __forceinline__ void reduce_tasks_grouped(const ReduceTasks& T, int n, double (*s_t)[2][4]) {
  const int tid = threadIdx.x, g = tid >> 8, lt = tid & 255, wv = (tid >> 6) & 3, lane = tid & 63;
  if (g < n) {
    const ReduceTask t = T.t[g];
    double v = 0.0;
    for (int r = lt; r < t.rows; r += 256) {
      const double x = t.src[(size_t)r * t.stride];
      v = t.is_max ? fmax(v, x) : v + x;
    }
    const double red = t.is_max ? wave_max(v) : wave_sum(v);
    double w = 0.0;
    for (int r = lt; r < t.rows2; r += 256) w += t.src2[r];
    const double red2 = wave_sum(w);
    if (lane == 0) { s_t[g][0][wv] = red; s_t[g][1][wv] = red2; }
  }
  __syncthreads();
  if (tid < n) {
    const ReduceTask t = T.t[tid];
    double total = t.is_max ? group4_max(s_t[tid][0]) : group4_sum(s_t[tid][0]);
    if (t.rows2 > 0) total += group4_sum(s_t[tid][1]);
    *t.out = total;
  }
  __syncthreads();
}

constexpr int kUpdImagesPerGroup = 42;
__device__ __forceinline__ void update_cameras_body(int vb, int NI, int NC, int cam_part, double radius, double dmin, double dmax,
                                                    const double* y, const double* scale_cam, const double* img_rec,
                                                    const double* cam_rec, const double* poses, const double* intr,
                                                    double* cand_poses, double* cand_intr, double* delta_cam, double* partial3,
                                                    double* cand_camrec, double* s_red) {
  const int i0 = vb * kUpdImagesPerGroup, i1 = min(i0 + kUpdImagesPerGroup, NI);
  double a_step = 0.0, a_model = 0.0, a_x2 = 0.0;
  auto one = [&](int t) {
    const double s = scale_cam[t];
    double n2, g, x;
    if (t < 6 * NI) {
      const int i = t / 6, e = t % 6;
      n2 = img_rec[(size_t)i * kImgRec + sym_idx(e, e, 6)]; g = img_rec[(size_t)i * kImgRec + 21 + e]; x = poses[t];
    } else {
      const int c = (t - 6 * NI) / 9, k = (t - 6 * NI) % 9;
      n2 = cam_rec[(size_t)c * kCamRec + sym_idx(k, k, 9)]; g = cam_rec[(size_t)c * kCamRec + 45 + k]; x = intr[9 * c + k];
    }
    double d = 0.0;
    if (s != 0.0) {
      const double yy = y[t];
      const double D2 = clampd(s * s * n2, dmin, dmax) / radius;
      d = -yy * s;
      if (cam_part) { a_model += 0.5 * yy * (s * g + D2 * yy); a_step += d * d; }
    }
    const double xn = x + d;
    if (s != 0.0 && cam_part) a_x2 += xn * xn;
    delta_cam[t] = d;
    if (t < 6 * NI) cand_poses[t] = xn; else cand_intr[t - 6 * NI] = xn;
  };
  for (int t = 6 * i0 + threadIdx.x; t < 6 * i1; t += 256) one(t);
  if (vb == 0)
    for (int t = 6 * NI + threadIdx.x; t < 6 * NI + 9 * NC; t += 256) one(t);
  const double s0 = block_sum_256(a_step, s_red);
  const double s1 = block_sum_256(a_model, s_red);
  const double s2 = block_sum_256(a_x2, s_red);
  if (threadIdx.x == 0) { partial3[3 * vb] = s0; partial3[3 * vb + 1] = s1; partial3[3 * vb + 2] = s2; }
  if (cand_camrec) {
    __syncthreads();
    for (int i = i0 + threadIdx.x; i < i1; i += 256) {
      double rec[9];
      cam_prepare(cand_poses + 6 * i, rec);
#pragma unroll
      for (int k = 0; k < 9; ++k) cand_camrec[9 * i + k] = rec[k];
    }
  }
}

__device__ __forceinline__ void lm_snapshot_body(int lane, const LmSpec& spec, double* dec, double* host_pub, double seq, double* fail_slots) {
  const LmDecision d = lm_decide(spec.scal, spec);
  if (lane == 0) { dec[0] = (double)d.code; dec[1] = d.radius; }
  volatile double* out = host_pub;
  double v = 0.0;
  if (lane < SC_COUNT) v = spec.scal[lane];
  else if (lane == SC_COUNT) v = (double)d.code;
  else if (lane == SC_COUNT + 1) v = d.radius;
  else if (lane == SC_COUNT + 2) v = d.decrease_factor;
  else if (lane == SC_COUNT + 3) v = d.rel;
  else if (lane == SC_COUNT + 4) v = d.step_norm;
  else if (lane == SC_COUNT + 5) v = d.cost_change;
  if (lane < SC_COUNT + 6) out[lane] = v;
  __threadfence_system();
  __builtin_amdgcn_wave_barrier();
  if (lane == 0) out[SC_COUNT + 7] = seq;
  if (lane < 2 && fail_slots) fail_slots[lane] = 0.0;
}

}
#endif
```

mavmap_amd/csrc/session.h:

```cpp
#ifndef MAVBA_SESSION_H_
#define MAVBA_SESSION_H_
#include <algorithm>
#include <chrono>
#include <cmath>
#include <cstdio>
#include <cstdlib>
#include <cstring>
#include <condition_variable>
#include <functional>
#include <limits>
#include <map>
#include <memory>
#include <mutex>
#include <shared_mutex>
#include <stdexcept>
#include <string>
#include <thread>
#include <unordered_map>
#include <vector>

#include "../../include/mavba.h"
#include "ba_math.h"
#include "internal.h"

// ... 181 lines not shown
static inline int model_k(int m) { return m == MAVBA_MODEL_PINHOLE ? 4 : m == MAVBA_MODEL_OPENCV ? 8 : 9; }
static inline int round_up(int x, int m) { return (x + m - 1) / m * m; }
static inline double now_s() {
  return std::chrono::duration<double>(std::chrono::steady_clock::now().time_since_epoch()).count();
}

struct KernelTimer { std::string name; long long launches = 0; double total_ms = 0.0; };

template <typename F>
static void parallel_ranges(long long n, F&& body, long long min_parallel = 200000) {
  int T = (int)std::min<long long>(host_threads(), std::max<long long>(n, 1));
  if (n < min_parallel) T = 1;
  if (T == 1) { body(0ll, n); return; }
  host_run(T, [&](int t) { body(n * t / T, n * (t + 1) / T); });
}

}

using namespace mavba;

struct mavba_session {
  mavba_options opt;
  int device = 0;
  hipStream_t st = nullptr;
  int NI = 0, NC = 0, NP = 0, N = 0, Nstride = 32, NPs = 32, KMAX = 4, n_full = 0, n_pad = 64, Q = 0;
  long long NO_all = 0;
  bool any_intr_free = false;
  std::vector<double> h_poses0, h_intr0, h_points0;
  std::vector<int> h_cam_model, h_img_cam, h_pt_start, h_oimg;
  std::vector<long long> perm;
  std::vector<int> h_pt_count_all;
  std::vector<double> h_dropped_rnorm;
  std::vector<double> h_dropped_cost;
  double fixed_cost_priors = 0.0;
  int num_priors_all = 0;
  std::vector<unsigned char> h_pt_removed;
  DevBuf<unsigned char> d_pt_active;
  std::vector<int> h_pt_orig;
  std::vector<unsigned char> h_pose_const, h_intr_const_in, h_pt_const_in;
  std::vector<unsigned char> h_img_used, h_cam_used, h_pt_used;
  std::vector<unsigned char> h_prior_on_img;
  std::vector<unsigned char> h_pose_free, h_intr_free, h_pt_free;
  double fixed_cost = 0.0;
  long long num_residuals = 0, num_residuals_reduced = 0, num_parameters_reduced = 0;
  int num_priors = 0;
  double prior_weight = 0.0;
  double setup_seconds = 0.0, solve_seconds = 0.0;

  DevBuf<double2> d_uv, d_im_uv;
  DevBuf<int> d_obs_img, d_obs_pt, d_pt_start, d_im_pt, d_img_cam, d_cam_model, d_img_chunk_start,
      d_cam_img_start, d_cam_imgs, d_prior_img, d_prior_start, d_q_pt, d_q_cam, d_q_start, d_pt_count;
  DevBuf<FrontTile> d_front_tiles;
  int num_front_tiles = 0;
  DevBuf<FrontTile> d_tail_tiles;
  int num_tail_tiles = 0, tail_begin = 0;
  bool front_ok = false;
  bool fused_ok = false;
  int eval_rows = 0;
  bool front_valid = false;
  double front_radius = 0.0;
  bool fail_slot_clean = false;
  bool planes_ready = false;
  DevBuf<SweepChunk> d_sweep_chunks;
  int num_sweep_chunks = 0;
  DevBuf<unsigned char> d_pose_free, d_intr_free, d_pt_free;
  DevBuf<double> d_prior_R0;
  DevBuf<SchurBlock> d_blocks;
  DevBuf<SchurChunk> d_chunks[3];
  DevBuf<SchurCluster> d_clusters;
  DevBuf<SchurRowsCluster> d_rows_clusters;
  DevBuf<int> d_rows_lists;
  DevBuf<unsigned> d_rows_emit;
  DevBuf<unsigned long long> d_rows_lanes;
  int rows_class_count[kRowsClasses] = {};
  bool rows_ok = false;
  bool rows_generic = false;
  DevBuf<PartialReduce> d_reduce_tasks;
  int num_reduce_tasks = 0;
  DevBuf<int> d_cl_tab, d_cl_lists;
  DevBuf<unsigned short> d_obs_meta, d_q_meta;
  DevBuf<unsigned char> d_pt_clustered;
  int num_clusters = 0, num_slots[3] = {0, 0, 0};
  ClusterShape cl_shape{16, 3};
  long long clustered_points = 0, cluster_partials = 0;
  double cluster_flops = 0.0;
  DevBuf<int2> d_terms[3];
  int num_blocks = 0, num_chunks[3] = {0, 0, 0};
  long long num_terms[3] = {0, 0, 0};
  DevBuf<double> d_poses, d_intr, d_points, d_cposes, d_cintr, d_cpoints, d_poses0, d_intr0, d_points0;
  DevBuf<double> d_camrec, d_ccamrec;
  bool camrec_current = false;
  DevBuf<double> d_R, d_Jp, d_Jc, d_Jk, d_Cu, d_gu, d_Gi, d_h, d_scale_cam, d_scale_pt;
  DevBuf<double> d_sweep_partial, d_camsum , d_img_intr_tmp, d_cam_partial;
  DevBuf<double> d_prior_res, d_prior_jac, d_prior_cost;
  DevBuf<double> d_Epose, d_Eintr, d_Wk, d_part[3];
  DevBuf<double> d_M, d_L, d_y, d_diag_ws, d_delta_cam, d_delta_pts, d_norm_partial, d_step_partial, d_scal;
  DevBuf<double> d_rnorm, d_perr;
  DevBuf<int> d_pt_orig;
  DevBuf<int> d_perm32;
  DevBuf<double> d_pts_out;
  double* d_img_rec = nullptr;
  double* d_cam_rec = nullptr;
  CholStructure chol_struct;
  bool prereduced = false;
  bool sweep_rode_along = false;
  bool setup_batched = false;
  bool M_is_clean = false;
  bool allow_persistent = true;
  bool persist_decided = false;
  bool speculate_on = true;
  void decide_persistent();
  int n_mat = 64, nd_parts = 0;
  std::vector<int> h_off_img, h_off_cam, h_col_var;
  DevBuf<int> d_off, d_col_var;
  DevBuf<double> d_ymat;
  DevBuf<int> d_ar_tiles;
  DevBuf<double> d_ar_buf;
  int num_ar_tiles = 0;

  bool evaluated = false, scales_ready = false, started = false, assembled = false;
  double radius = 1e4, decrease_factor = 2.0;
  double cost = 0.0, x_norm = 0.0, grad_max = 0.0, abs_gtol = 0.0, initial_cost = 0.0;
  int iteration = 0, invalid_steps = 0, n_success = 0, n_fail = 0;
  int termination = MAVBA_TERM_RUNNING;

  mavba_allreduce_fn ar_fn = nullptr;
  void* ar_ctx = nullptr;
  void* rccl_comm = nullptr;
  bool rccl_comm_owned = true;
  std::shared_ptr<RcclGuard> rccl_guard;
  bool sharded() const { return (ar_fn || rccl_comm) && (world > 1 || force_exchange); }
  bool force_exchange = false;
  int rank = 0, world = 1;

  std::vector<KernelTimer> timers;
  struct Pending { int idx; hipEvent_t a, b; bool own_a = true; };
  std::vector<Pending> pending;
  std::vector<hipEvent_t> ev_pool;

  ~mavba_session() {
    if (st) (void)hipStreamSynchronize(st);
    if (rccl_comm && rccl_comm_owned) rccl_comm_destroy(rccl_comm);
    if (lm_pub) lm_pub_free(lm_pub);
    HostSpare<long long>::give(perm); HostSpare<int>::give(h_oimg); HostSpare<double>::give(h_points0);
    for (auto& p : pending) { (void)hipEventDestroy(p.a); (void)hipEventDestroy(p.b); }
    for (auto& e : ev_pool) (void)hipEventDestroy(e);
    if (st) stream_release(st, device);
  }

// ... 47 lines not shown
        rccl_allreduce(rccl_comm, dptr, count, op, st);
      } else {
        rccl_allreduce(rccl_comm, dptr, count, op, st);
      }
      return;
    }
    sync();
    if (ar_fn(ar_ctx, dptr, count, op) != 0) throw Failure(MAVBA_ERR_HIP, "all-reduce hook failed");
  }

  SweepArgs sweep_args(const double* camrec, const double* intr, const double* points) {
    SweepArgs a;
    a.N = N; a.Nstride = Nstride; a.NI = NI; a.NC = NC; a.KMAX = KMAX;
    a.uv = d_uv.p; a.obs_img = d_obs_img.p; a.obs_pt = d_obs_pt.p;
    a.camrec = camrec; a.intr = intr; a.img_cam = d_img_cam.p; a.cam_model = d_cam_model.p;
    a.points = points;
    a.pt_active = h_pt_removed.empty() ? nullptr : d_pt_active.p;
    a.loss_b = opt.loss_scale_factor * opt.loss_scale_factor; a.loss_inv_b = 1.0 / a.loss_b;
    a.R = d_R.p; a.Jp = d_Jp.p; a.Jc = d_Jc.p; a.Jk = d_Jk.p; a.cost_partial = d_sweep_partial.p;
    return a;
  }
  void read_scalars(double* h) {
    HIP_OK(hipMemcpyAsync(h, d_scal.p, SC_COUNT * sizeof(double), hipMemcpyDeviceToHost, st));
    sync();
  }

  void build(const mavba_problem* P, const DeviceRaw* raw = nullptr);
void intr_entries_on_device(const std::vector<unsigned char>& cam_active, std::vector<int>& q_start, std::vector<int>& q_cam);
    void order_on_device(const mavba_problem* P, std::vector<int>& img_start, const DeviceRaw* raw);
  void order_on_host(const mavba_problem* P, const long long* keptp, std::vector<int>& img_start,
                     std::unique_ptr<PinnedBuf<double2>>& uv_h, std::unique_ptr<PinnedBuf<int>>& opt_h,
                     std::unique_ptr<PinnedBuf<double2>>& im_uv_h, std::unique_ptr<PinnedBuf<int>>& im_pt_h);
  void ensure_perm_host();
  void derive_free_flags();
  void finish_structure();
  void choose_elimination_order(const std::vector<SchurBlock>& blocks);
  void reset_state();
  void evaluate(double next_radius = -1.0);
  void evaluate_enqueue(double next_radius = -1.0, const LmSpec& spec = lm_spec_off());
  void launch_front(double r, bool entries, const LmSpec& spec = lm_spec_off(), const CamSweepArgs* with_sweep = nullptr);
  DevBuf<double> d_lm_dec;
  double* lm_pub = nullptr;
  double lm_seq = 0.0;
  LmSpec lm_spec(bool pending_eval) const {
    LmSpec sp{};
    sp.dec = nullptr; sp.scal = d_scal.p;
    sp.radius = radius; sp.decrease_factor = decrease_factor;
    sp.ptol = opt.parameter_tolerance; sp.ftol = opt.function_tolerance; sp.min_rel_dec = opt.min_relative_decrease;
    sp.max_radius = opt.max_trust_region_radius; sp.abs_gtol = abs_gtol; sp.pending_eval = pending_eval ? 1 : 0;
    return sp;
  }
  bool wait_publication(double* h);
  void build_front_tiles(const std::vector<int>& q_start);
  void build_tiles(const std::vector<int>& q_start, int first, DevBuf<FrontTile>& out, int& count);
  void ensure_planes();
  bool fused_now() const { return fused_ok && rows_ok; }
  int eval_cost_rows() const { return front_ok ? eval_rows : (N > 0 ? jacobian_sweep_grid(N) : 0); }
  void take_evaluation(const double* h) { cost = h[SC_COST]; grad_max = h[SC_GRAD_MAX]; x_norm = std::sqrt(h[SC_XNORM2]); }
  void assemble(double r);
  void solve_linear(double r);
  void linear_step(double r, double* h_scal);
  void candidate(double r, double* h_scal);
  void candidate_enqueue(double r, ReduceTasks* tail = nullptr, int* tail_count = nullptr);
  bool merge_small() const;
  bool merge_on = true;
  double pub_wait_seconds = 0.0;
  bool cameras_updated = false;
  double cameras_updated_r = 0.0;
  void start();
  int iterate(int max_iters, int* done);
  void point_errors(double* out);
  void restart();
  long long filter_points(double max_error, const unsigned char* keep, unsigned char* removed_out, double* errors_out);
  void restore_initial_params() {
    HIP_OK(hipMemcpyAsync(d_poses.p, d_poses0.p, (size_t)NI * 6 * 8, hipMemcpyDeviceToDevice, st));
    HIP_OK(hipMemcpyAsync(d_intr.p, d_intr0.p, (size_t)NC * 9 * 8, hipMemcpyDeviceToDevice, st));
    HIP_OK(hipMemcpyAsync(d_points.p, d_points0.p, (size_t)NP * 3 * 8, hipMemcpyDeviceToDevice, st));
    camrec_current = false; evaluated = false; front_valid = false;
  }
  void apply_filter_state();
  void to_caller_points(const double* internal, double* out, int width) const {
    for (int q = 0; q < NP; ++q)
      for (int e = 0; e < width; ++e) out[(size_t)h_pt_orig[q] * width + e] = internal[(size_t)q * width + e];
  }
  void fill_result(mavba_result* r);
};
#endif
```

mavmap_amd/csrc/session_build.hip:

```cpp
#include "session.h"
#include <array>
#include <map>

using namespace mavba;


void mavba_session::derive_free_flags() {
  h_pose_free.assign((size_t)NI * 6, 0);
  h_intr_free.assign((size_t)NC * 9, 0);
  h_pt_free.assign(NP, 0);
  for (int i = 0; i < NI; ++i) {
    if (!h_img_used[i]) continue;
    const unsigned m = h_pose_const[i];
    for (int e = 0; e < 6; ++e) {
      const bool c = e < 3 ? (m & MAVBA_CONST_RVEC) != 0 : (m & (MAVBA_CONST_TX << (e - 3))) != 0;
      h_pose_free[(size_t)i * 6 + e] = c ? 0 : 1;
    }
  }
  any_intr_free = false;
  for (int c = 0; c < NC; ++c) {
    if (!h_cam_used[c] || h_intr_const_in[c]) continue;
    for (int k = 0; k < model_k(h_cam_model[c]); ++k) h_intr_free[(size_t)c * 9 + k] = 1;
    any_intr_free = true;
  }
// ... 333 lines not shown
  img_chunk_start[NI] = (int)sweep_chunks.size();
  num_sweep_chunks = (int)sweep_chunks.size();
  std::vector<int> cam_img_start(NC + 1, 0), cam_imgs(std::max(NI, 1));
  for (int i = 0; i < NI; ++i) cam_img_start[h_img_cam[i] + 1]++;
  for (int c = 0; c < NC; ++c) cam_img_start[c + 1] += cam_img_start[c];
  {
    std::vector<int> cur(cam_img_start.begin(), cam_img_start.end() - 1);
    for (int i = 0; i < NI; ++i) cam_imgs[cur[h_img_cam[i]]++] = i;
  }
  std::vector<int> prior_img(num_priors), prior_start(NI + 1, 0);
  std::vector<double> prior_R0((size_t)num_priors * 9);
  for (int k = 0; k < num_priors; ++k) {
    prior_img[k] = pri[k].first;
    prior_start[pri[k].first + 1]++;
    rot_matrix_colmajor(&P->rot_prior_rvec[3 * pri[k].second], &prior_R0[(size_t)k * 9]);
  }
  for (int i = 0; i < NI; ++i) prior_start[i + 1] += prior_start[i];

  n_full = 6 * NI + 9 * NC;
  n_pad = std::max(64, round_up(n_full, 64));

  lap("image-major view");
  if (!device_order) {
    d_uv.upload_pinned(uv_h->data(), (size_t)N, st); d_obs_img.upload(h_oimg, st); d_obs_pt.upload_pinned(opt_h->data(), (size_t)N, st); d_pt_start.upload(h_pt_start, st);
    d_im_uv.upload_pinned(im_uv_h->data(), (size_t)N, st); d_im_pt.upload_pinned(im_pt_h->data(), (size_t)N, st);
  }
  d_img_cam.upload(h_img_cam, st); d_cam_model.upload(h_cam_model, st);
  d_sweep_chunks.upload(sweep_chunks, st); d_img_chunk_start.upload(img_chunk_start, st);
  d_cam_img_start.upload(cam_img_start, st); d_cam_imgs.upload(cam_imgs, st);
  d_prior_img.upload(prior_img, st); d_prior_start.upload(prior_start, st); d_prior_R0.upload(prior_R0, st);
  d_pt_count.upload(h_pt_count_all, st);
  if (!device_order) { d_pt_orig.upload(h_pt_orig, st); d_points0.upload(h_points0, st); }
  d_pts_out.alloc((size_t)std::max(NP, 1) * 3);
  d_poses0.upload(h_poses0, st); d_intr0.upload(h_intr0, st);
  const size_t nI = std::max(NI, 1), nC = std::max(NC, 1), nP = std::max(NP, 1);
  d_poses.alloc(nI * 6); d_intr.alloc(nC * 9); d_points.alloc(nP * 3);
  d_cposes.alloc(nI * 6); d_cintr.alloc(nC * 9); d_cpoints.alloc(nP * 3);
  d_camrec.alloc(nI * 9); d_ccamrec.alloc(nI * 9);
  d_Cu.alloc((size_t)6 * NPs); d_gu.alloc((size_t)3 * NPs); d_Gi.alloc((size_t)6 * NPs); d_h.alloc((size_t)3 * NPs);
  d_Gi.zero(st); d_h.zero(st);
  d_scale_cam.alloc((size_t)n_pad); d_scale_pt.alloc((size_t)3 * NPs);
  d_scale_cam.zero(st); d_scale_pt.zero(st);
  d_sweep_partial.alloc((size_t)std::max(jacobian_sweep_grid(std::max(N, 1)), kFrontMaxGrid) + 8);
  d_camsum.alloc(nI * kImgRec + nC * kCamRec);
  d_camsum.zero(st);
  d_img_rec = d_camsum.p; d_cam_rec = d_camsum.p + (size_t)NI * kImgRec;
  d_img_intr_tmp.alloc(nI * kCamRec);
  d_cam_partial.alloc((size_t)std::max(num_sweep_chunks, 1) * kSweepAcc);
  d_prior_res.alloc(std::max(num_priors, 1)); d_prior_jac.alloc((size_t)std::max(num_priors, 1) * 3);
  d_prior_cost.alloc(std::max(num_priors, 1));
  d_Epose.alloc((size_t)std::max(N, 1) * kPoseRec);
  d_y.alloc(n_pad); d_y.zero(st);
  d_delta_cam.alloc(n_pad); d_delta_pts.alloc(nP * 3);
  d_norm_partial.alloc((size_t)(512 + kStateNormsCamBlocks) * 2); d_step_partial.alloc((size_t)(1024 + update_cameras_groups(NI) + 2) * 3);
  d_scal.alloc(SC_COUNT); d_scal.zero(st);
  d_rnorm.alloc(std::max(N, 1)); d_perr.alloc(nP);

  lap("alloc + upload");
  derive_free_flags();
  finish_structure();
  lap("finish_structure total");
  setup_batched = false;
  if (batch.open) { batch.open = false; HIP_OK(upload_batch_end(true)); }
  reset_state();
  sync();
  lap("reset + sync");
  setup_seconds = now_s() - t0;
}

namespace mavba {
std::vector<ElimNode> elimination_tree(int NI, int NC, const std::vector<std::vector<int>>& lower, int forced, int max_depth) {
  std::vector<ElimNode> tn;
  typedef ElimNode TNode;
  {
    const int tail = 9 * NC;
    auto tiles_of = [](int cols) { return (cols + 63) / 64; };
    if (forced > 1) {
      std::vector<int> cut(forced);
      for (int q = 0; q < forced; ++q) cut[q] = (int)((long long)q * NI / forced);
      std::vector<std::vector<int>> part(forced);
      std::vector<int> sep;
      int run = 0;
      for (int i = 0; i < NI; ++i) {
        while (run + 1 < forced && i >= cut[run + 1]) ++run;
        int m = i;
        for (int c : lower[i]) m = std::min(m, c);
        if (m < cut[run]) sep.push_back(i); else part[run].push_back(i);
      }
      int np = 0;
      for (auto& pr : part) if (!pr.empty()) { tn.push_back(TNode{std::move(pr), -1}); ++np; }
      if (np >= 2) {
        for (auto& t : tn) t.parent = np;
        tn.push_back(TNode{std::move(sep), -1});
      } else {
        tn.clear();
      }
    } else {
      std::vector<std::vector<int>> adj(NI);
      for (int r = 0; r < NI; ++r)
        for (int c : lower[r]) { adj[r].push_back(c); adj[c].push_back(r); }
      for (auto& a : adj) { std::sort(a.begin(), a.end()); a.erase(std::unique(a.begin(), a.end()), a.end()); }
      bool use_levels = true;
      if (const char* e = std::getenv("MAVBA_ND_LEVELS")) use_levels = std::atoi(e) != 0;
      std::vector<int> pos(NI, -1), level(NI, -1);
      std::function<std::pair<int, int>(std::vector<int>&&, int, int)> rec = [&](std::vector<int>&& M, int depth, int tl) {
        const int n = (int)M.size();
// ... 227 lines not shown
void mavba_session::finish_structure() {
  const bool tt = std::getenv("MAVBA_SETUP_TIMING") != nullptr;
  double tl = now_s();
  auto lap = [&](const char* what) { if (tt) { const double t = now_s(); std::fprintf(stderr, "[setup]   %-26s %8.2f ms\n", what, 1e3 * (t - tl)); tl = t; } };
  d_pose_free.upload(h_pose_free, st); d_intr_free.upload(h_intr_free, st); d_pt_free.upload(h_pt_free, st);
  std::vector<unsigned char> img_active(NI, 0), cam_active(NC, 0);
  for (int i = 0; i < NI; ++i) for (int e = 0; e < 6; ++e) img_active[i] |= h_pose_free[(size_t)i * 6 + e];
  for (int c = 0; c < NC; ++c) for (int k = 0; k < 9; ++k) cam_active[c] |= h_intr_free[(size_t)c * 9 + k];

  std::vector<int> q_start(NP + 1, 0), q_pt, q_cam;
  bool q_on_device = false;
  {
    bool any_cam_active = false;
    for (int c = 0; c < NC; ++c) any_cam_active |= cam_active[c] != 0;
    auto cams_of = [&](int p, int* out) {
      int n = 0;
      for (int a = h_pt_start[p]; a < h_pt_start[p + 1]; ++a) {
        const int c = h_img_cam[h_oimg[a]];
        if (!cam_active[c]) continue;
        int k = 0;
        while (k < n && out[k] != c) ++k;
        if (k == n) out[n++] = c;
      }
      std::sort(out, out + n);
      return n;
    };
    const char* setup_env = std::getenv("MAVBA_SETUP");
    const bool q_host = setup_env && std::string(setup_env) == "host";
    q_on_device = any_cam_active && N >= 50000 && !q_host;
    if (q_on_device) {
      intr_entries_on_device(cam_active, q_start, q_cam);
    } else if (any_cam_active) {
      parallel_ranges(NP, [&](long long p0, long long p1) {
        std::vector<int> tmp(std::max(NC, 1));
        for (long long p = p0; p < p1; ++p) q_start[p + 1] = h_pt_free[p] ? cams_of((int)p, tmp.data()) : 0;
      }, 20000);
      for (int p = 0; p < NP; ++p) q_start[p + 1] += q_start[p];
      q_pt.resize((size_t)q_start[NP]); q_cam.resize((size_t)q_start[NP]);
      parallel_ranges(NP, [&](long long p0, long long p1) {
        std::vector<int> tmp(std::max(NC, 1));
        for (long long p = p0; p < p1; ++p) {
          if (q_start[p + 1] == q_start[p]) continue;
          const int n = cams_of((int)p, tmp.data());
          for (int k = 0; k < n; ++k) { q_pt[(size_t)q_start[p] + k] = (int)p; q_cam[(size_t)q_start[p] + k] = tmp[k]; }
        }
      }, 20000);
    }
  }
  Q = (int)q_cam.size();
  if (!q_on_device) { d_q_start.upload(q_start, st); d_q_pt.upload(q_pt, st); d_q_cam.upload(q_cam, st); }
  d_Eintr.alloc((size_t)std::max(Q, 1) * kIntrRec);
  if (planes_ready) d_Wk.alloc((size_t)std::max(Q, 1) * 27);
  build_front_tiles(q_start);

  lap("flags + intr entries");
  std::vector<unsigned char> pt_mode(NP, 0);
  std::vector<unsigned short> obs_meta((size_t)std::max(N, 1), 0xFFFFu), q_meta((size_t)std::max(Q, 1), 0xFFFFu);
  std::vector<SchurCluster> clusters;
  std::vector<int> cl_imgs, cl_cams;
  {
    cl_shape = ClusterShape{16, 3};
    if (const char* e = std::getenv("MAVBA_CLUSTER_SHAPE")) cl_shape = std::atoi(e) == 12 ? ClusterShape{12, 2} : ClusterShape{16, 3};
  }
  tail_begin = NP;
  while (tail_begin > 0 && (h_pt_start[tail_begin] - h_pt_start[tail_begin - 1] > kTailObs || h_pt_const_in[tail_begin - 1])) --tail_begin;
  const ClusterShape sh = cl_shape;
  const int kClTab = sh.tab(), kClTabPP = sh.tab_pp(), kClTabIP = sh.tab_ip(), kClTabII = sh.tab_ii();
  const int kClImages = sh.images, kClCams = sh.cams;
  std::vector<int> cl_ni, cl_nc, cl_kr;
  auto cam_rows_of = [&](const std::vector<int>& cams) { int k = 0; for (int c : cams) k += model_k(h_cam_model[c]); return k; };
  const bool no_fuse_env = std::getenv("MAVBA_NO_FUSE") != nullptr;
  auto build_clusters = [&](bool rows_mode) {
    clusters.clear(); cl_imgs.clear(); cl_cams.clear(); cl_ni.clear(); cl_nc.clear(); cl_kr.clear();
    std::fill(pt_mode.begin(), pt_mode.end(), 0);
    bool use_clusters = true;
    if (const char* e = std::getenv("MAVBA_CLUSTERS")) use_clusters = std::atoi(e) != 0;
    long long nfree = 0;
    for (int p = 0; p < NP; ++p) nfree += h_pt_free[p] != 0;
    int kMaxPoints = (int)std::min<long long>(256, std::max<long long>(kClBatch, round_up((int)(nfree / 512), kClBatch)));
    if (rows_mode) kMaxPoints = (int)std::min<long long>(kRowsMaxPoints, std::max<long long>(nfree <= 4096 ? kRowsBatch : 2 * kRowsBatch, round_up((int)(nfree / 1024), kRowsBatch)));
    if (const char* e = std::getenv("MAVBA_CLUSTER_POINTS")) kMaxPoints = std::max(1, std::atoi(e));
    if (rows_mode) kMaxPoints = std::min(kMaxPoints, kRowsMaxPoints);
    double kCostF = 20000.0, kCostB[kRowsClasses] = {15400.0, 17500.0, 27500.0};
    if (const char* e = std::getenv("MAVBA_ROWS_COST")) std::sscanf(e, "%lf,%lf,%lf,%lf", &kCostF, &kCostB[0], &kCostB[1], &kCostB[2]);
    const int kRange = 2048;
    const int nranges = (NP + kRange - 1) / kRange;
    std::vector<std::vector<SchurCluster>> r_clusters(nranges);
    std::vector<std::vector<int>> r_imgs(nranges), r_cams(nranges), r_ni(nranges), r_nc(nranges), r_kr(nranges);
    auto do_range = [&](int rg, std::vector<int>& in_cluster, std::vector<int>& in_point) {
      const int r0 = rg * kRange, r_end = std::min(NP, r0 + kRange);
      for (int p = std::max(r0, tail_begin); p < r_end; ++p)
        if (h_pt_free[p] && (h_pt_start[p + 1] > h_pt_start[p] || q_start[p + 1] > q_start[p])) pt_mode[p] = 2;
      const int r1 = std::min(r_end, std::max(r0, tail_begin));
      std::vector<int> cur_i, cur_c, pi;
      int cl_serial = rg * (kRange + 1);
      int cur_p0 = r0, cur_n = 0;
      auto close = [&](int p_end) {
        if (cur_n > 0) {
          r_ni[rg].push_back((int)cur_i.size()); r_nc[rg].push_back((int)cur_c.size()); r_kr[rg].push_back(cam_rows_of(cur_c));
          std::sort(cur_i.begin(), cur_i.end());
          std::sort(cur_c.begin(), cur_c.end());
          r_clusters[rg].push_back(SchurCluster{cur_p0, p_end});
          for (int k = 0; k < kClImages; ++k) r_imgs[rg].push_back(k < (int)cur_i.size() ? cur_i[k] : -1);
          for (int k = 0; k < kClCams; ++k) r_cams[rg].push_back(k < (int)cur_c.size() ? cur_c[k] : -1);
        }
        cur_i.clear(); cur_c.clear(); cur_n = 0; cur_p0 = p_end; ++cl_serial;
// ... 503 lines not shown
      d_rows_clusters.upload(rc, st);
      d_rows_emit.upload(emit_all, st);
      std::vector<int> rl((size_t)std::max(num_clusters, 1) * kRowsLists, -1);
      for (int c = 0; c < num_clusters; ++c) {
        const int o = order[c];
        int* L = &rl[(size_t)c * kRowsLists];
        for (int k = 0; k < kClImages; ++k) { const int img = cl_imgs[(size_t)o * kClImages + k]; L[k] = img; L[kRowsListsCam + k] = img >= 0 ? h_img_cam[img] : -1; }
        for (int k = 0; k < kClCams; ++k) L[kRowsListsCams + k] = cl_cams[(size_t)o * kClCams + k];
      }
      d_rows_lists.upload(rl, st);
      if (std::getenv("MAVBA_CLUSTER_STATS")) {
        long long pts[kRowsClasses] = {}, bat[kRowsClasses] = {};
        for (int c = 0; c < num_clusters; ++c) { const int k = row_class(order[c]); pts[k] += rc[c].p1 - rc[c].p0; bat[k] += (rc[c].p1 - rc[c].p0 + kRowsBatch - 1) / kRowsBatch; }
        for (int k = 0; k < kRowsClasses; ++k)
          std::fprintf(stderr, "[cluster stats] k_schur_rows class %d (%d rows): %d clusters, %lld points, %lld batches\n", k, 16 * kRowsClassNT[k], rows_class_count[k], pts[k], bat[k]);
        long long hist[kClImagesMax + 1][kClCamsMax + 1][2] = {}, unplaced = 0;
        for (int c = 0; c < num_clusters; ++c) { hist[rc[c].ni][rc[c].nc][0]++; hist[rc[c].ni][rc[c].nc][1] += (rc[c].p1 - rc[c].p0 + kRowsBatch - 1) / kRowsBatch; unplaced += (rc[c].flags & kRowsUnplaced) != 0; }
        std::fprintf(stderr, "[cluster stats] k_schur_rows clusters / batches by (images, cameras):");
        for (int i = 0; i <= kClImagesMax; ++i) for (int k = 0; k <= kClCamsMax; ++k) if (hist[i][k][0]) std::fprintf(stderr, " (%d,%d) %lld/%lld", i, k, hist[i][k][0], hist[i][k][1]);
        std::fprintf(stderr, "; clusters that keep the selects: %lld\n", unplaced);
      }
    }
    std::vector<SchurCluster> cl_sorted(clusters.size());
    std::vector<int> tab_sorted(cl_tab.size(), -1);
    std::vector<int> lists_sorted((size_t)std::max(num_clusters, 1) * (kClImages + kClCams), -1);
    for (int c = 0; c < num_clusters; ++c) {
      cl_sorted[c] = clusters[order[c]];
      std::copy(cl_tab.begin() + (size_t)order[c] * kClTab, cl_tab.begin() + (size_t)(order[c] + 1) * kClTab, tab_sorted.begin() + (size_t)c * kClTab);
    }
    for (int c = 0; c < num_clusters; ++c) {
      std::copy(cl_imgs.begin() + (size_t)order[c] * kClImages, cl_imgs.begin() + (size_t)(order[c] + 1) * kClImages, lists_sorted.begin() + (size_t)c * (kClImages + kClCams));
      std::copy(cl_cams.begin() + (size_t)order[c] * kClCams, cl_cams.begin() + (size_t)(order[c] + 1) * kClCams, lists_sorted.begin() + (size_t)c * (kClImages + kClCams) + kClImages);
    }
    d_clusters.upload(cl_sorted, st); d_cl_tab.upload(tab_sorted, st); d_cl_lists.upload(lists_sorted, st);
    d_obs_meta.upload(obs_meta, st); d_q_meta.upload(q_meta, st); d_pt_clustered.upload(ptc, st);
  }
  {
    long long head_observed = 0, head_clustered = 0;
    for (int p = 0; p < tail_begin; ++p) { head_observed += h_pt_start[p + 1] > h_pt_start[p]; head_clustered += pt_mode[p] == 1; }
    const bool no_fuse = std::getenv("MAVBA_NO_FUSE") != nullptr;
    fused_ok = front_ok && !no_fuse && cl_shape.images == 16 && num_clusters > 0 && head_clustered == head_observed &&
               clustered_points == head_clustered && num_clusters <= kFrontMaxGrid;
    num_tail_tiles = 0;
    if (fused_ok && h_pt_start[NP] > h_pt_start[tail_begin]) {
      build_tiles(q_start, tail_begin, d_tail_tiles, num_tail_tiles);
      if ((long long)num_clusters + point_front_grid(num_tail_tiles) > kFrontMaxGrid) { fused_ok = false; num_tail_tiles = 0; }
    }
    rows_ok = rows_ok && fused_ok;
  }
  if (!setup_batched) sync();
  lap("upload terms");
}

void mavba_session::build_front_tiles(const std::vector<int>& q_start) {
  const bool planes_only = std::getenv("MAVBA_FRONT_PLANES") != nullptr;
  front_ok = !planes_only;
  for (int p = 0; p < NP && front_ok; ++p)
    if (q_start[p + 1] - q_start[p] > kFrontQ) front_ok = false;
  num_front_tiles = 0;
  if (front_ok) build_tiles(q_start, 0, d_front_tiles, num_front_tiles);
  else d_front_tiles.upload(std::vector<FrontTile>(), st);
  front_valid = false;
  if (!front_ok) ensure_planes();
}
void mavba_session::build_tiles(const std::vector<int>& q_start, int first, DevBuf<FrontTile>& out, int& count) {
  std::vector<FrontTile> tiles;
  int p0 = first, obs = 0, qs = 0;
  for (int p = first; p < NP; ++p) {
    const int c = h_pt_start[p + 1] - h_pt_start[p], nq = q_start[p + 1] - q_start[p];
    if (p > p0 && (obs + c > kFrontObs || p - p0 >= kFrontPts || qs + nq > kFrontQ)) {
      tiles.push_back(FrontTile{p0, p, h_pt_start[p0], h_pt_start[p], q_start[p0], q_start[p]});
      p0 = p; obs = 0; qs = 0;
    }
    obs += c; qs += nq;
  }
  if (NP > p0) tiles.push_back(FrontTile{p0, NP, h_pt_start[p0], h_pt_start[NP], q_start[p0], q_start[NP]});
  count = (int)tiles.size();
  out.upload(tiles, st);
}

void mavba_session::reset_state() {
  front_valid = false;
  if (!h_pt_removed.empty()) {
    h_pt_removed.clear();
    apply_filter_state();
    M_is_clean = false;
  }
  HIP_OK(hipMemcpyAsync(d_poses.p, d_poses0.p, (size_t)NI * 6 * 8, hipMemcpyDeviceToDevice, st));
  HIP_OK(hipMemcpyAsync(d_intr.p, d_intr0.p, (size_t)NC * 9 * 8, hipMemcpyDeviceToDevice, st));
  HIP_OK(hipMemcpyAsync(d_points.p, d_points0.p, (size_t)NP * 3 * 8, hipMemcpyDeviceToDevice, st));
  evaluated = scales_ready = started = assembled = false;
  camrec_current = false;
  radius = opt.initial_trust_region_radius; decrease_factor = 2.0;
  cost = x_norm = grad_max = abs_gtol = initial_cost = 0.0;
  iteration = invalid_steps = n_success = n_fail = 0;
  termination = MAVBA_TERM_RUNNING;
  solve_seconds = 0.0;
}
```

mavmap_amd/csrc/session_lm.hip:

```cpp
#include "session.h"
#include "lm_decide.h"
#if defined(__x86_64__) || defined(__i386__)
#include <immintrin.h>
#define MAVBA_CPU_RELAX() _mm_pause()
#else
#include <thread>
#define MAVBA_CPU_RELAX() std::this_thread::yield()
#endif

using namespace mavba;


void mavba_session::ensure_planes() {
  if (planes_ready) return;
  d_R.alloc((size_t)2 * Nstride); d_Jp.alloc((size_t)6 * Nstride); d_Jc.alloc((size_t)12 * Nstride);
  d_Jk.alloc((size_t)2 * KMAX * Nstride);
  d_Wk.alloc((size_t)std::max(Q, 1) * 27);
  planes_ready = true;
}

void mavba_session::launch_front(double r, bool entries, const LmSpec& spec, const CamSweepArgs* with_sweep) {
  sweep_rode_along = false;
  prereduced = false;
  FrontArgs f;
// ... 166 lines not shown
                                 d_scale_pt.p, d_Gi.p, d_h.p, d_Epose.p, d_pt_start.p, d_Cu.p, d_gu.p, r, dmin, dmax,
                                 d_scal.p + SC_FAIL);
    });
    timed("entries_intr", [&] {
      launch_entries_intr(st, Q, NI, NPs, d_q_pt.p, d_q_cam.p, d_Wk.p, d_scale_cam.p, d_scale_pt.p, d_Gi.p, d_h.p,
                          d_Eintr.p);
    });
  }
  if (!M_is_clean) {
    timed("memset_S", [&] {
      HIP_OK(hipMemsetAsync(d_M.p, 0, chol_struct.store_doubles() * sizeof(double), st));
      launch_fix_diag(st, n_mat, chol_struct.d_tile_slot, rank == 0, d_col_var.p, d_scale_cam.p, d_M.p);
    });
    M_is_clean = true;
  }
  if (!(front_ok && fused_now())) timed("schur_clusters", [&] {
    launch_schur_clusters(st, cl_shape, num_clusters, d_clusters.p, d_cl_tab.p, d_pt_start.p, d_q_start.p, d_obs_meta.p,
                          d_q_meta.p, d_pt_clustered.p, d_Epose.p, d_Eintr.p, d_h.p, NPs, d_part[0].p, d_part[1].p,
                          d_part[2].p);
  });
  if (num_chunks[0] > 0) timed("schur_chunks_pp", [&] { launch_schur_chunks(st, BLK_PP, num_chunks[0], d_chunks[0].p, d_terms[0].p, d_Epose.p, d_Eintr.p, d_part[0].p); });
  if (num_chunks[1] > 0) timed("schur_chunks_ip", [&] { launch_schur_chunks(st, BLK_IP, num_chunks[1], d_chunks[1].p, d_terms[1].p, d_Epose.p, d_Eintr.p, d_part[1].p); });
  if (num_chunks[2] > 0) timed("schur_chunks_ii", [&] { launch_schur_chunks(st, BLK_II, num_chunks[2], d_chunks[2].p, d_terms[2].p, d_Epose.p, d_Eintr.p, d_part[2].p); });
  const int nbt = n_mat / 64;
  timed("schur_finalize", [&] {
    if (!(prereduced && front_valid && front_radius == r)) launch_partial_reduce(st, num_reduce_tasks, d_reduce_tasks.p, d_part[0].p, d_part[1].p, d_part[2].p);
    launch_schur_finalize(st, num_blocks, d_blocks.p, d_part[0].p, d_part[1].p, d_part[2].p, NI, NC, chol_struct.d_tile_slot, nbt, rank == 0,
                          r, dmin, dmax, d_img_cam.p, d_img_rec, d_cam_rec, d_scale_cam.p, d_off.p, d_off.p + NI, d_M.p);
  });
  if (sharded()) {
    launch_tiles_copy(st, num_ar_tiles, d_ar_tiles.p, chol_struct.d_tile_slot, nbt, d_M.p, d_ar_buf.p, true);
    allreduce(d_ar_buf.p, (long long)num_ar_tiles * 4096 + n_mat, 0);
    launch_tiles_copy(st, num_ar_tiles, d_ar_tiles.p, chol_struct.d_tile_slot, nbt, d_M.p, d_ar_buf.p, false);
  }
  assembled = true;
}

void mavba_session::decide_persistent() {
  if (persist_decided) return;
  if (chol_struct.persist_ok && !sharded()) allow_persistent = persistent_allowed_now();
  persist_decided = true;
}

void mavba_session::solve_linear(double r) {
  decide_persistent();
  assemble(r);
  CamUpdateArgs u;
  const bool with_update = merge_small();
  if (with_update) {
    u.NI = NI; u.NC = NC; u.cam_part = rank == 0 ? 1 : 0; u.radius = r; u.dmin = opt.min_lm_diagonal; u.dmax = opt.max_lm_diagonal;
    u.scale_cam = d_scale_cam.p; u.img_rec = d_img_rec; u.cam_rec = d_cam_rec; u.poses = d_poses.p; u.intr = d_intr.p;
    u.cand_poses = d_cposes.p; u.cand_intr = d_cintr.p; u.delta_cam = d_delta_cam.p;
    u.partial3 = d_step_partial.p + 3 * (size_t)backsub_points_grid(NP); u.cand_camrec = d_ccamrec.p;
  }
  timed_split("chol_factor", "chol_backsolve", [&](hipEvent_t mid) {
    cameras_updated = dense_spd_solve_device(st, d_M.p, n_mat, d_ymat.p, d_scal.p + SC_FAIL, d_diag_ws.p, d_L.p, chol_struct, d_col_var.p, d_y.p,
                                             allow_persistent, mid, with_update ? &u : nullptr);
    cameras_updated_r = r;
  });
  assembled = false;
  fail_slot_clean = false;
  if (!(allow_persistent && chol_struct.persist_ok) || sharded()) M_is_clean = false;
}

void mavba_session::linear_step(double r, double* h) {
  solve_linear(r);
  candidate(r, h);
  if (h[SC_FAIL] >= 1e29 && allow_persistent) {
    std::fprintf(stderr, "mavba: persistent factorisation timed out, falling back to the launch-per-panel schedule\n");
    allow_persistent = false;
    persistent_timed_out();
    solve_linear(r);
    candidate(r, h);
  }
}

void mavba_session::candidate(double r, double* h) {
  candidate_enqueue(r);
  read_scalars(h);
}
void mavba_session::candidate_enqueue(double r, ReduceTasks* tail, int* tail_count) {
  const double dmin = opt.min_lm_diagonal, dmax = opt.max_lm_diagonal;
  const int rows = backsub_points_grid(NP), ugroups = update_cameras_groups(NI);
  if (!(cameras_updated && cameras_updated_r == r))
    timed("update_cameras", [&] {
      launch_update_cameras(st, NI, NC, rank == 0, r, dmin, dmax, d_y.p, d_scale_cam.p, d_img_rec, d_cam_rec,
                            d_poses.p, d_intr.p, d_cposes.p, d_cintr.p, d_delta_cam.p, d_step_partial.p + 3 * (size_t)rows,
                            d_ccamrec.p);
    });
  cameras_updated = false;
  static const long long fuse_max_obs = [] { const char* e = std::getenv("MAVBA_COST_FUSE_MAX_OBS"); return e ? std::atoll(e) : 500000ll; }();
  const bool cost_separate = (long long)N > fuse_max_obs;
  timed("backsub_points", [&] {
    launch_backsub_points_jvp(st, NP, NPs, NI, r, dmin, dmax, sweep_args(d_camrec.p, d_intr.p, d_points.p), d_pt_start.p,
                              d_delta_cam.p, d_pt_free.p, d_Gi.p, d_h.p, d_Cu.p, d_gu.p, d_scale_pt.p, d_cpoints.p,
                              d_delta_pts.p, d_step_partial.p, d_ccamrec.p, d_cintr.p, cost_separate ? nullptr : d_sweep_partial.p);
  });
  SweepArgs a = sweep_args(d_ccamrec.p, d_cintr.p, d_cpoints.p);
  if (cost_separate) timed("cost_only", [&] { launch_cost_only(st, a); });
  if (num_priors > 0)
    timed("rot_prior", [&] {
      launch_rot_prior(st, num_priors, d_prior_img.p, d_prior_R0.p, prior_weight, d_cposes.p, d_prior_res.p,
                       d_prior_jac.p, d_prior_cost.p);
    });
  {
    const int nsweep = N > 0 ? (cost_separate ? jacobian_sweep_grid(N) : rows) : 0;
    ReduceTasks T;
    T.t[0] = ReduceTask{d_step_partial.p, rows + ugroups, 3, 0, nullptr, 0, d_scal.p + SC_STEP_NORM2};
    T.t[1] = ReduceTask{d_step_partial.p + 1, rows + ugroups, 3, 0, nullptr, 0, d_scal.p + SC_MODEL_CHANGE};
    T.t[2] = ReduceTask{d_step_partial.p + 2, rows + ugroups, 3, 0, nullptr, 0, d_scal.p + SC_CAND_XNORM2};
    T.t[3] = ReduceTask{d_sweep_partial.p, nsweep, 1, 0, d_prior_cost.p, num_priors, d_scal.p + SC_NEW_COST};
    if (tail) { *tail = T; *tail_count = 4; }
    else timed("reduce", [&] { launch_reduce_tasks(st, T, 4); });
  }
  if (sharded()) allreduce(d_scal.p + SC_CAND_BEGIN, SC_CAND_COUNT, 0);
}

bool mavba_session::merge_small() const {
  return merge_on && !sharded() && NI <= 64 && NC <= 8 && NP <= 8192 && dense_spd_solve_is_small(n_mat, chol_struct);
}

void mavba_session::start() {
  { const char* e = std::getenv("MAVBA_MERGE"); merge_on = !e || std::atoi(e) != 0; }
  { const char* e = std::getenv("MAVBA_SPECULATE"); speculate_on = !e || std::atoi(e) != 0; }
  decide_persistent();
  evaluate();
  initial_cost = cost + fixed_cost;
  const double g0 = std::max(grad_max, std::numeric_limits<double>::epsilon());
  abs_gtol = opt.gradient_tolerance * g0;
  started = true;
  if (num_residuals_reduced == 0 || num_parameters_reduced == 0) { termination = MAVBA_TERM_FUNCTION_TOLERANCE; return; }
  if (grad_max <= abs_gtol) { termination = MAVBA_TERM_GRADIENT_TOLERANCE; return; }
  if (opt.print_progress) {
    std::printf("%4s %14s %12s %10s %10s %10s %10s\n", "iter", "cost", "cost_change", "|gradient|", "|step|", "tr_ratio", "tr_radius");
    std::printf("%4d %14.6e %12.2e %10.2e %10.2e %10.2e %10.2e\n", 0, cost + fixed_cost, 0.0, grad_max, 0.0, 0.0, radius);
  }
}

bool mavba_session::wait_publication(double* h) {
  volatile double* pub = lm_pub;
  const double t_end = now_s() + 2.0;
  for (long long spin = 0;; ++spin) {
    if (pub[SC_COUNT + 7] == lm_seq) break;
    MAVBA_CPU_RELAX();
    if ((spin & 0xFFFF) == 0xFFFF && now_s() > t_end) return false;
  }
  std::atomic_thread_fence(std::memory_order_acquire);
  for (int i = 0; i < SC_COUNT; ++i) h[i] = pub[i];
// ... 234 lines not shown
```

Before: 1302 iter/s.

## Tile back-substitution by point observation counts and precompute per-image step records

Points are grouped on the host into tiles of at most 64 observations or 64 points. The back-substitution kernel is rewritten to work per wavefront over these tiles, with a separate path for long tiles, prefetched gathers and a launch-bounds occupancy hint. The camera update kernel now writes a per-image rotated step record once, so each observation no longer recomputes the cross products from the camera delta. The default observation limit for fusing the cost into back-substitution is raised, so this 2M-observation problem now takes the fused path. In exchange the change adds a tile table, a new per-image buffer, more kernel complexity, and a build hook that rebuilds and adjusts the timestamp of an oracle reference shim.

Result: no change. 1303 iter/s (median of 3 runs) (+0.1%).

```diff
diff --git a/include/mavba.h b/include/mavba.h
--- a/include/mavba.h
+++ b/include/mavba.h
@@ -211,6 +211,8 @@
 int mavba_debug_elimination_tree(int32_t num_images, int32_t num_cameras, int64_t npairs, const int32_t* pair_a,
                                  const int32_t* pair_b, int32_t max_depth, int32_t* node_of_image, int32_t* node_parent,
                                  int32_t cap);
+
+int mavba_debug_backsub_tiles(int32_t num_points, const int32_t* pt_start, int32_t* tiles, int32_t cap);
 
 int mavba_debug_radix_sort(int32_t n, const uint32_t* keys, int32_t key_bytes, int32_t* order_out, int32_t device);
 int64_t mavba_debug_upload_batch(int32_t n, const int64_t* sizes, int64_t arena_bytes, int32_t device);
diff --git a/mavmap_amd/__init__.py b/mavmap_amd/__init__.py
--- a/mavmap_amd/__init__.py
+++ b/mavmap_amd/__init__.py
@@ -1,4 +1,4 @@
 from . import _abi
 from .problem import BAProblem
 from .api import (BundleAdjustmentOptions, MavbaError, Scene, Session, bundle_adjustment,
-                  bundle_adjustment_filter_rebundle, pose_refinement, pose_refinement_batch, device_count, dense_spd_solve, rccl_unique_id, load, lib_path, radix_sort_order, elimination_tree, debug_upload_batch)
+                  bundle_adjustment_filter_rebundle, pose_refinement, pose_refinement_batch, device_count, dense_spd_solve, rccl_unique_id, load, lib_path, radix_sort_order, elimination_tree, debug_upload_batch, backsub_tiles)
diff --git a/mavmap_amd/api.py b/mavmap_amd/api.py
--- a/mavmap_amd/api.py
+++ b/mavmap_amd/api.py
@@ -22,7 +22,7 @@
     "mavba_scene_get_camera", "mavba_scene_flatten", "mavba_scene_bundle_adjust",
     "mavba_rccl_unique_id", "mavba_session_set_rccl", "mavba_pose_refine_batch", "mavba_session_set_params", "mavba_session_restart", "mavba_session_filter_points", "mavba_solve_filter_solve",
     "mavba_debug_elimination_tree", "mavba_debug_radix_sort", "mavba_debug_lm_decide", "mavba_debug_chol_schedule",
-    "mavba_debug_inproc_comms", "mavba_debug_upload_batch",
+    "mavba_debug_inproc_comms", "mavba_debug_upload_batch", "mavba_debug_backsub_tiles",
 ]
 
 ALLREDUCE_FN = C.CFUNCTYPE(C.c_int, C.c_void_p, C.c_void_p, C.c_int64, C.c_int32)
@@ -100,6 +100,7 @@
     L.mavba_session_filter_points.argtypes = [sp, C.c_double, bp, bp, dp, C.POINTER(C.c_int64)]
     L.mavba_solve_filter_solve.argtypes = [pp, op, C.c_double, bp, rp, rp, dp, bp, C.POINTER(C.c_int64)]
     L.mavba_debug_elimination_tree.argtypes = [C.c_int32, C.c_int32, C.c_int64, ip, ip, C.c_int32, ip, ip, C.c_int32]
+    L.mavba_debug_backsub_tiles.argtypes = [C.c_int32, ip, ip, C.c_int32]
     L.mavba_debug_radix_sort.argtypes = [C.c_int32, C.POINTER(C.c_uint32), C.c_int32, ip, C.c_int32]
     L.mavba_debug_lm_decide.argtypes = [C.c_int32, dp, dp, dp, C.c_int32]
     i32p, i64p = C.POINTER(C.c_int32), C.POINTER(C.c_int64)
@@ -511,6 +512,18 @@
     return node[:num_images], parent[:n]
 
 
+def backsub_tiles(pt_start):
+    ps = np.ascontiguousarray(pt_start, dtype=np.int32)
+    if ps.ndim != 1 or len(ps) < 1:
+        raise ValueError("pt_start needs num_points + 1 entries")
+    n = len(ps) - 1
+    tiles = np.zeros((max(n, 1), 4), np.int32)
+    k = load().mavba_debug_backsub_tiles(n, A.ptr(ps, C.c_int32), A.ptr(tiles, C.c_int32), len(tiles))
+    if k < 0:
+        _check(k)
+    return tiles[:k].copy()
+
+
 def radix_sort_order(keys, key_bytes=4, device=-1):
     keys = np.ascontiguousarray(keys, dtype=np.uint32)
     out = np.zeros(len(keys), np.int32)
diff --git a/mavmap_amd/build.py b/mavmap_amd/build.py
--- a/mavmap_amd/build.py
+++ b/mavmap_amd/build.py
@@ -74,7 +74,33 @@
         import json
         with open(STAMP, "w") as fh:
             json.dump(dict(digest=source_digest()), fh)
+    refresh_reference_shim()
     return LIB
+
+
+REPO = os.path.dirname(ROOT)
+REFERENCE_SHIM = os.path.join(REPO, "oracle", "_ref", "_shim_mock_reffm.so")
+REFERENCE_SHIM_DEPS = [os.path.join(REPO, *f) for f in (("tests", "shim", "shim_driver.cpp"), ("tests", "shim", "mock_mavba.cpp"),
+                                                        ("shim", "base3d", "bundle_adjustment.cc"), ("shim", "base3d", "bundle_adjustment.h"),
+                                                        ("include", "mavba.h"))]
+
+
+def refresh_reference_shim():
+    oracle = os.path.join(REPO, "oracle")
+    if not os.path.exists(os.path.join(oracle, "Makefile")) or shutil.which("make") is None:
+        return
+    mtime = lambda f: os.stat(f).st_mtime_ns
+    before = mtime(REFERENCE_SHIM) if os.path.exists(REFERENCE_SHIM) else None
+    subprocess.check_call(["make", "-C", oracle, "-s", "ref"], stdout=subprocess.DEVNULL)
+    if not os.path.exists(REFERENCE_SHIM):
+        return
+    newest = max(mtime(d) for d in REFERENCE_SHIM_DEPS if os.path.exists(d))
+    if mtime(REFERENCE_SHIM) >= newest:
+        return
+    if mtime(REFERENCE_SHIM) != before:
+        os.utime(REFERENCE_SHIM, ns=(newest, newest))
+    else:
+        os.remove(REFERENCE_SHIM)
 
 
 if __name__ == "__main__":
diff --git a/mavmap_amd/csrc/api.hip b/mavmap_amd/csrc/api.hip
--- a/mavmap_amd/csrc/api.hip
+++ b/mavmap_amd/csrc/api.hip
@@ -345,6 +345,19 @@
     for (int i : tn[t].imgs) node_of_image[i] = (int)t;
   }
   return (int)tn.size();
+  MAVBA_CATCH
+}
+
+int mavba_debug_backsub_tiles(int32_t NP, const int32_t* pt_start, int32_t* tiles, int32_t cap) {
+  MAVBA_TRY
+  if (NP < 0 || !pt_start || cap < 0 || (cap > 0 && !tiles)) throw Failure(MAVBA_ERR_INVALID_ARGUMENT, "bad argument");
+  if (pt_start[0] != 0) throw Failure(MAVBA_ERR_INVALID_ARGUMENT, "pt_start must begin with 0");
+  for (int p = 0; p < NP; ++p)
+    if (pt_start[p + 1] < pt_start[p]) throw Failure(MAVBA_ERR_INVALID_ARGUMENT, "pt_start must not decrease");
+  const std::vector<BacksubTile> t = build_backsub_tiles(NP, pt_start);
+  if ((int)t.size() > cap) throw Failure(MAVBA_ERR_INVALID_ARGUMENT, "tiles too small");
+  for (size_t k = 0; k < t.size(); ++k) { tiles[4 * k] = t[k].p0; tiles[4 * k + 1] = t[k].p1; tiles[4 * k + 2] = t[k].o0; tiles[4 * k + 3] = t[k].o1; }
+  return (int)t.size();
   MAVBA_CATCH
 }
 
diff --git a/mavmap_amd/csrc/ba_math.h b/mavmap_amd/csrc/ba_math.h
--- a/mavmap_amd/csrc/ba_math.h
+++ b/mavmap_amd/csrc/ba_math.h
@@ -243,25 +243,36 @@
   }
 }
 
-MAVBA_HD void obs_backsub_term(int model, const double* rec, const double* cam, const double* X, double uo, double vo,
-                               const double* dc, const double* dk, double* r, double* t) {
+MAVBA_HD void image_step_record(const double* rec, const double* dc, double* step) {
+  const double b = rec[7], c = rec[8];
+  double m1[3], m2[3];
+  cross3(rec, dc, m1);
+  cross3(rec, m1, m2);
+  step[0] = dc[0] + b * m1[0] + c * m2[0]; step[1] = dc[1] + b * m1[1] + c * m2[1]; step[2] = dc[2] + b * m1[2] + c * m2[2];
+  step[3] = dc[3]; step[4] = dc[4]; step[5] = dc[5];
+}
+MAVBA_HD void obs_backsub_term_step(int model, const double* rec, const double* cam, const double* X, double uo, double vo,
+                                    const double* step, const double* dk, double* r, double* t) {
   double Xr[3], Xc[3], u, v, A[6], tk0, tk1;
   transform_point(rec, X, Xr, Xc);
   project_dk(model, cam, Xc, dk, u, v, A, tk0, tk1);
   r[0] = u - uo; r[1] = v - vo;
-  const double a = rec[6], b = rec[7], c = rec[8];
-  double m1[3], m2[3], om[3], dX[3];
-  cross3(rec, dc, m1);
-  cross3(rec, m1, m2);
-  om[0] = dc[0] + b * m1[0] + c * m2[0]; om[1] = dc[1] + b * m1[1] + c * m2[1]; om[2] = dc[2] + b * m1[2] + c * m2[2];
-  cross3(om, Xr, dX);
-  dX[0] += dc[3]; dX[1] += dc[4]; dX[2] += dc[5];
+  const double a = rec[6], b = rec[7];
+  double m1[3], m2[3], dX[3];
+  cross3(step, Xr, dX);
+  dX[0] += step[3]; dX[1] += step[4]; dX[2] += step[5];
   const double tau0 = A[0] * dX[0] + A[1] * dX[1] + A[2] * dX[2] + tk0;
   const double tau1 = A[3] * dX[0] + A[4] * dX[1] + A[5] * dX[2] + tk1;
   const double q[3] = {A[0] * tau0 + A[3] * tau1, A[1] * tau0 + A[4] * tau1, A[2] * tau0 + A[5] * tau1};
   cross3(rec, q, m1);
   cross3(rec, m1, m2);
   t[0] = q[0] - a * m1[0] + b * m2[0]; t[1] = q[1] - a * m1[1] + b * m2[1]; t[2] = q[2] - a * m1[2] + b * m2[2];
+}
+MAVBA_HD void obs_backsub_term(int model, const double* rec, const double* cam, const double* X, double uo, double vo,
+                               const double* dc, const double* dk, double* r, double* t) {
+  double step[6];
+  image_step_record(rec, dc, step);
+  obs_backsub_term_step(model, rec, cam, X, uo, vo, step, dk, r, t);
 }
 
 MAVBA_HD void cauchy_weight(double s, double b, double inv_b, double& w, double& half_rho) {
diff --git a/mavmap_amd/csrc/dense_chol.hip b/mavmap_amd/csrc/dense_chol.hip
--- a/mavmap_amd/csrc/dense_chol.hip
+++ b/mavmap_amd/csrc/dense_chol.hip
@@ -175,11 +175,6 @@
 constexpr int kFuseTasks = 256;
 constexpr int kMaxBacksolveGroups = 2048;
 
-__device__ __forceinline__ void wave_lds_sync() {
-  __builtin_amdgcn_fence(__ATOMIC_RELEASE, "wavefront");
-  __builtin_amdgcn_wave_barrier();
-  __builtin_amdgcn_fence(__ATOMIC_ACQUIRE, "wavefront");
-}
 
 struct NoPhaseHook { __device__ __forceinline__ void operator()(int) const {} };
 struct NoMark { __device__ __forceinline__ void operator()(int) const {} };
@@ -2252,7 +2247,7 @@
     const int groups = (U.NI + kUpdImagesPerGroup - 1) / kUpdImagesPerGroup;
     for (int vb = 0; vb < (groups > 0 ? groups : 1); ++vb) {
       update_cameras_body(vb, U.NI, U.NC, U.cam_part, U.radius, U.dmin, U.dmax, y_nat, U.scale_cam, U.img_rec, U.cam_rec, U.poses, U.intr,
-                          U.cand_poses, U.cand_intr, U.delta_cam, U.partial3, U.cand_camrec, s_red);
+                          U.cand_poses, U.cand_intr, U.delta_cam, U.partial3, U.cand_camrec, U.camrec, U.img_step, s_red);
       __syncthreads();
     }
   }
diff --git a/mavmap_amd/csrc/dev_reduce.h b/mavmap_amd/csrc/dev_reduce.h
--- a/mavmap_amd/csrc/dev_reduce.h
+++ b/mavmap_amd/csrc/dev_reduce.h
@@ -3,6 +3,12 @@
 #include <hip/hip_runtime.h>
 
 namespace mavba {
+
+__device__ __forceinline__ void wave_lds_sync() {
+  __builtin_amdgcn_fence(__ATOMIC_RELEASE, "wavefront");
+  __builtin_amdgcn_wave_barrier();
+  __builtin_amdgcn_fence(__ATOMIC_ACQUIRE, "wavefront");
+}
 
 __device__ __forceinline__ double wave_sum(double v) {
 #define MAVBA_ROR_ADD(N)                                                                                   \
diff --git a/mavmap_amd/csrc/internal.h b/mavmap_amd/csrc/internal.h
--- a/mavmap_amd/csrc/internal.h
+++ b/mavmap_amd/csrc/internal.h
@@ -231,8 +231,12 @@
                      const double* scale_cam, double* S);
 
 int backsub_points_grid(int NP);
+struct BacksubTile { int p0, p1, o0, o1; };
+std::vector<BacksubTile> build_backsub_tiles(int NP, const int* pt_start);
 void launch_backsub_points_jvp(hipStream_t st, int NP, int NPs, int NI, double radius, double dmin, double dmax,
-                               const SweepArgs& a, const int* pt_start, const double* delta_cam,
+                               const SweepArgs& a, const int* pt_start, const BacksubTile* tiles, int num_tiles,
+                               const int* long_tiles , int num_long,
+                               const double* img_step, const double* delta_cam,
                                const unsigned char* pt_free, const double* Gi, const double* h, const double* Cu,
                                const double* gu, const double* scale_pt, double* cand_points, double* delta_points,
                                double* partial , const double* cand_camrec = nullptr, const double* cand_intr = nullptr,
@@ -242,7 +246,8 @@
                            double dmax, const double* y, const double* scale_cam,
                            const double* img_rec, const double* cam_rec, const double* poses,
                            const double* intr, double* cand_poses, double* cand_intr,
-                           double* delta_cam, double* partial3 , double* cand_camrec );
+                           double* delta_cam, double* partial3 , double* cand_camrec ,
+                           const double* camrec , double* img_step );
 
 void launch_reduce_cols(hipStream_t st, const double* partial, int rows, int cols, int stride,
                         unsigned max_mask, double* out, bool accumulate);
@@ -357,6 +362,7 @@
   int NI, NC, cam_part; double radius, dmin, dmax;
   const double* scale_cam; const double* img_rec; const double* cam_rec; const double* poses; const double* intr;
   double* cand_poses; double* cand_intr; double* delta_cam; double* partial3; double* cand_camrec;
+  const double* camrec; double* img_step;
 };
 bool dense_spd_solve_is_small(int n_pad, const CholStructure& cs);
 bool dense_spd_solve_device(hipStream_t st, double* M, int n_pad, double* y, double* fail,
diff --git a/mavmap_amd/csrc/kernels.hip b/mavmap_amd/csrc/kernels.hip
--- a/mavmap_amd/csrc/kernels.hip
+++ b/mavmap_amd/csrc/kernels.hip
@@ -1527,26 +1527,40 @@
 }
 
 constexpr int kBsCamsLds = 16;
-__global__ void __launch_bounds__(256) k_backsub_points_packed(
-    int NP, int NPs, int NI, int NC, int N, int ppb, int nblocks, double radius, double dmin, double dmax, double loss_b, double loss_inv_b,
-    const int* __restrict__ pt_start, const int* __restrict__ obs_img, const int* __restrict__ obs_pt,
-    const double2* __restrict__ uv, const int* __restrict__ img_cam, const int* __restrict__ cam_model,
-    const double* __restrict__ camrec, const double* __restrict__ intr, const double* __restrict__ delta_cam,
+constexpr int kBsWaves = 4;
+#ifndef MAVBA_BS_SKIP
+#define MAVBA_BS_SKIP 0
+#endif
+#ifndef MAVBA_BS_PREFETCH
+#define MAVBA_BS_PREFETCH 2
+#endif
+#ifndef MAVBA_BS_MIN_WAVES
+#define MAVBA_BS_MIN_WAVES 2
+#endif
+template <bool CAMS_LDS>
+__global__ void __launch_bounds__(256, MAVBA_BS_MIN_WAVES) k_backsub_points(
+    int NP, int NPs, int NI, int NC, int N, int num_tiles, int num_long, double radius, double dmin, double dmax, double loss_b, double loss_inv_b,
+    const BacksubTile* __restrict__ tiles, const int* __restrict__ long_tiles, const int* __restrict__ pt_start, const int* __restrict__ obs_img,
+    const int* __restrict__ obs_pt, const double2* __restrict__ uv, const int* __restrict__ img_cam,
+    const int* __restrict__ cam_model, const double* __restrict__ camrec, const double* __restrict__ intr,
+    const double* __restrict__ img_step, const double* __restrict__ delta_cam,
     const unsigned char* __restrict__ pt_free, const double* __restrict__ Gi, const double* __restrict__ h,
     const double* __restrict__ Cu, const double* __restrict__ gu, const double* __restrict__ scale_pt,
     const double* __restrict__ points, double* __restrict__ cand_points, double* __restrict__ delta_points,
     double* __restrict__ partial, const double* __restrict__ cand_camrec, const double* __restrict__ cand_intr,
     const unsigned char* __restrict__ pt_active, double* __restrict__ cost_partial) {
-  __shared__ double s_t[3][256];
-  __shared__ double s_new[3][128];
+  __shared__ double s_t[kBsWaves][3][64];
+  __shared__ double s_new[kBsWaves][3][64];
   __shared__ double s_red[4];
   __shared__ double s_kin[kBsCamsLds][9], s_dk[kBsCamsLds][9];
   __shared__ int s_model[kBsCamsLds];
-  const int tid = threadIdx.x;
-  const bool cams_lds = NC <= kBsCamsLds;
+  const int tid = threadIdx.x, lane = tid & 63;
+  const int wv = __builtin_amdgcn_readfirstlane(tid >> 6);
   double a_step = 0.0, a_model = 0.0, a_x2 = 0.0, a_cost = 0.0;
-  const int G = (int)gridDim.x;
+  const int S = (int)gridDim.x * kBsWaves;
   struct Obs { int pt, im; double2 m; };
+  struct GatherPt { double X[3]; int cam; bool fr; };
+  struct GatherIm { double rec[9], step[6]; };
   auto load_obs = [&](int o) {
     Obs r{0, 0, make_double2(0.0, 0.0)};
     if (N <= 0) return r;
@@ -1554,142 +1568,195 @@
     r.pt = obs_pt[oc]; r.im = obs_img[oc]; r.m = uv[oc];
     return r;
   };
-  auto obs_term = [&](const Obs& q, bool valid, double (&t)[3]) {
+  auto gather_pt = [&](const Obs& q, bool valid) {
+    GatherPt g;
+    g.X[0] = g.X[1] = g.X[2] = 0.0; g.cam = 0; g.fr = false;
+    if (valid) {
+      g.fr = pt_free[q.pt] != 0;
+      g.cam = img_cam[q.im];
+#pragma unroll
+      for (int k = 0; k < 3; ++k) g.X[k] = points[3 * (size_t)q.pt + k];
+    }
+    return g;
+  };
+  auto gather_im = [&](const Obs& q, bool valid) {
+    GatherIm g;
+#pragma unroll
+    for (int k = 0; k < 9; ++k) g.rec[k] = 0.0;
+#pragma unroll
+    for (int k = 0; k < 6; ++k) g.step[k] = 0.0;
+    if (valid) {
+#pragma unroll
+      for (int k = 0; k < 9; ++k) g.rec[k] = camrec[9 * q.im + k];
+#pragma unroll
+      for (int k = 0; k < 6; ++k) g.step[k] = img_step[6 * q.im + k];
+    }
+    return g;
+  };
+  auto obs_term = [&](const Obs& q, const GatherPt& g, const GatherIm& gi, bool valid, double (&t)[3]) {
     t[0] = t[1] = t[2] = 0.0;
-    if (!valid || !pt_free[q.pt]) return;
-    const int cam = img_cam[q.im];
-    const double X[3] = {points[3 * (size_t)q.pt], points[3 * (size_t)q.pt + 1], points[3 * (size_t)q.pt + 2]};
-    double rec[9], kin[9], dc[6], dk[9];
-#pragma unroll
-    for (int k = 0; k < 9; ++k) rec[k] = camrec[9 * q.im + k];
-#pragma unroll
-    for (int k = 0; k < 6; ++k) dc[k] = delta_cam[6 * q.im + k];
-    int model;
-    if (cams_lds) {
-      model = s_model[cam];
-#pragma unroll
-      for (int k = 0; k < 9; ++k) { kin[k] = s_kin[cam][k]; dk[k] = s_dk[cam][k]; }
-    } else {
-      model = cam_model[cam];
-#pragma unroll
-      for (int k = 0; k < 9; ++k) { kin[k] = intr[9 * cam + k]; dk[k] = delta_cam[6 * NI + 9 * cam + k]; }
-    }
+    if (!valid || !g.fr) return;
+    const double* kin = CAMS_LDS ? s_kin[g.cam] : intr + 9 * g.cam;
+    const double* dk = CAMS_LDS ? s_dk[g.cam] : delta_cam + 6 * NI + 9 * g.cam;
+    const int model = CAMS_LDS ? s_model[g.cam] : cam_model[g.cam];
     double r[2], tt[3];
-#ifndef MAVBA_BS_SKIP
-#define MAVBA_BS_SKIP 0
-#endif
-    if (MAVBA_BS_SKIP & 1) { r[0] = rec[0] + kin[0] + dc[0] + dk[0]; r[1] = X[0] + q.m.x; tt[0] = rec[3]; tt[1] = X[1]; tt[2] = q.m.y; }
+    if (MAVBA_BS_SKIP & 1) { r[0] = gi.rec[0] + kin[0] + gi.step[0] + dk[0]; r[1] = g.X[0] + q.m.x; tt[0] = gi.rec[3]; tt[1] = g.X[1]; tt[2] = q.m.y; }
     else
-    obs_backsub_term(model, rec, kin, X, q.m.x, q.m.y, dc, dk, r, tt);
+    obs_backsub_term_step(model, gi.rec, kin, g.X, q.m.x, q.m.y, gi.step, dk, r, tt);
     double w, half_rho;
     cauchy_weight(r[0] * r[0] + r[1] * r[1], loss_b, loss_inv_b, w, half_rho);
     const double w2 = w * w;
     t[0] = w2 * tt[0]; t[1] = w2 * tt[1]; t[2] = w2 * tt[2];
   };
-  int o0 = 0, o1 = 0, o0n = 0, o1n = 0;
-  Obs cur{0, 0, make_double2(0.0, 0.0)};
-  if ((int)blockIdx.x < nblocks) {
-    const int b0 = (int)blockIdx.x;
-    o0 = pt_start[b0 * ppb]; o1 = pt_start[min(b0 * ppb + ppb, NP)];
-    if (b0 + G < nblocks) { o0n = pt_start[(b0 + G) * ppb]; o1n = pt_start[min((b0 + G) * ppb + ppb, NP)]; }
-    cur = load_obs(o0 + tid);
-  }
-  if (cams_lds) {
-    for (int e = tid; e < 9 * NC; e += 256) { s_kin[e / 9][e % 9] = intr[e]; s_dk[e / 9][e % 9] = delta_cam[6 * NI + e]; }
-    for (int c = tid; c < NC; c += 256) s_model[c] = cam_model[c];
-    __syncthreads();
-  }
-  for (int blk = blockIdx.x; blk < nblocks; blk += G) {
-    const int p0 = blk * ppb, p1 = min(p0 + ppb, NP);
-    const int p = p0 + tid;
-    const bool owner = p < p1;
-    int o0nn = 0, o1nn = 0;
-    Obs nxt = cur;
-    if (blk + G < nblocks) {
-      nxt = load_obs(o0n + tid);
-      if (blk + 2 * G < nblocks) { o0nn = pt_start[(blk + 2 * G) * ppb]; o1nn = pt_start[min((blk + 2 * G) * ppb + ppb, NP)]; }
-    }
-    int mb = 0, me = 0;
-    bool fr = false;
-    double G[6] = {0, 0, 0, 0, 0, 0}, sp[3] = {0, 0, 0}, hh[3] = {0, 0, 0}, cu[3] = {0, 0, 0}, gg[3] = {0, 0, 0}, Xo[3] = {0, 0, 0};
-    if (owner) {
-      mb = pt_start[p]; me = pt_start[p + 1];
-      fr = pt_free[p] != 0;
-#pragma unroll
-      for (int k = 0; k < 3; ++k) Xo[k] = points[3 * (size_t)p + k];
-      if (fr) {
-        const int dg[3] = {0, 3, 5};
-#pragma unroll
-        for (int k = 0; k < 6; ++k) G[k] = Gi[k * NPs + p];
-#pragma unroll
-        for (int k = 0; k < 3; ++k) { sp[k] = scale_pt[k * NPs + p]; hh[k] = h[k * NPs + p]; cu[k] = Cu[dg[k] * NPs + p]; gg[k] = gu[k * NPs + p]; }
-      }
-    }
+  struct Owner { bool fr; double G[6], sp[3], hh[3], cu[3], gg[3], Xo[3]; };
+  auto load_owner = [&](int p) {
+    Owner w;
+    w.fr = pt_free[p] != 0;
+#pragma unroll
+    for (int k = 0; k < 6; ++k) w.G[k] = 0.0;
+#pragma unroll
+    for (int k = 0; k < 3; ++k) { w.Xo[k] = points[3 * (size_t)p + k]; w.sp[k] = w.hh[k] = w.cu[k] = w.gg[k] = 0.0; }
+    if (w.fr) {
+      const int dg[3] = {0, 3, 5};
+#pragma unroll
+      for (int k = 0; k < 6; ++k) w.G[k] = Gi[k * NPs + p];
+#pragma unroll
+      for (int k = 0; k < 3; ++k) { w.sp[k] = scale_pt[k * NPs + p]; w.hh[k] = h[k * NPs + p]; w.cu[k] = Cu[dg[k] * NPs + p]; w.gg[k] = gu[k * NPs + p]; }
+    }
+    return w;
+  };
+  auto owner_update = [&](int p, const Owner& w, const double (&T)[3], int slot) {
+    double d[3] = {0, 0, 0};
+    if (w.fr) {
+      const double q0 = -w.sp[0] * T[0], q1 = -w.sp[1] * T[1], q2 = -w.sp[2] * T[2];
+      const double z[3] = {q0 * w.G[0], q0 * w.G[1] + q1 * w.G[2], q0 * w.G[3] + q1 * w.G[4] + q2 * w.G[5]};
+      const double tt[3] = {w.hh[0] - z[0], w.hh[1] - z[1], w.hh[2] - z[2]};
+      double yp[3];
+      git_mul(w.G, tt, yp);
+#pragma unroll
+      for (int k = 0; k < 3; ++k) {
+        const double s = w.sp[k];
+        const double D2 = clampd(s * s * w.cu[k], dmin, dmax) / radius;
+        const double gs = s * w.gg[k];
+        a_model += 0.5 * yp[k] * (gs + D2 * yp[k]);
+        d[k] = -yp[k] * s;
+        a_step += d[k] * d[k];
+      }
+    }
+#pragma unroll
+    for (int k = 0; k < 3; ++k) {
+      const double xn = w.Xo[k] + d[k];
+      cand_points[3 * (size_t)p + k] = xn;
+      delta_points[3 * (size_t)p + k] = d[k];
+      if (w.fr) a_x2 += xn * xn;
+      if (cost_partial) s_new[wv][k][slot] = xn;
+    }
+  };
+  auto cand_cost = [&](const Obs& c, int cam, int slot) {
+    double r[2];
+    const double Xn[3] = {s_new[wv][0][slot], s_new[wv][1][slot], s_new[wv][2][slot]};
+    obs_residual(CAMS_LDS ? s_model[cam] : cam_model[cam], cand_camrec + 9 * c.im, cand_intr + 9 * cam, Xn, c.m.x, c.m.y, r);
+    double w, half_rho;
+    cauchy_weight(r[0] * r[0] + r[1] * r[1], loss_b, loss_inv_b, w, half_rho);
+    if (pt_active && !pt_active[c.pt]) half_rho = 0.0;
+    a_cost += half_rho;
+  };
+  const BacksubTile none{0, 0, 0, 0};
+  const int t_first = (int)blockIdx.x * kBsWaves + wv;
+  {
+    int t = t_first;
+    BacksubTile T0 = none, T1 = none, T2 = none;
+    Obs cur{0, 0, make_double2(0.0, 0.0)}, nxt = cur;
+    if (t < num_tiles) { T0 = tiles[t]; cur = load_obs(T0.o0 + lane); }
+    if (t + S < num_tiles) { T1 = tiles[t + S]; nxt = load_obs(T1.o0 + lane); }
+    if (t + 2 * S < num_tiles) T2 = tiles[t + 2 * S];
+    GatherPt gcur = gather_pt(cur, T0.o0 + lane < T0.o1);
+#if MAVBA_BS_PREFETCH >= 2
+    GatherIm icur = gather_im(cur, T0.o0 + lane < T0.o1);
+#endif
+    if (CAMS_LDS) {
+      for (int e = tid; e < 9 * NC; e += 256) { s_kin[e / 9][e % 9] = intr[e]; s_dk[e / 9][e % 9] = delta_cam[6 * NI + e]; }
+      for (int c = tid; c < NC; c += 256) s_model[c] = cam_model[c];
+      __syncthreads();
+    }
+    for (; t < num_tiles; t += S) {
+      BacksubTile T3 = none;
+      if (t + 3 * S < num_tiles) T3 = tiles[t + 3 * S];
+      Obs nn = nxt;
+      if (t + 2 * S < num_tiles) nn = load_obs(T2.o0 + lane);
+#if MAVBA_BS_PREFETCH >= 1
+      const GatherPt gnxt = gather_pt(nxt, T1.o0 + lane < T1.o1);
+#else
+      gcur = gather_pt(cur, T0.o0 + lane < T0.o1);
+#endif
+#if MAVBA_BS_PREFETCH >= 2
+      const GatherIm inxt = gather_im(nxt, T1.o0 + lane < T1.o1);
+#else
+      const GatherIm icur = gather_im(cur, T0.o0 + lane < T0.o1);
+#endif
+      const int p0 = T0.p0, o0 = T0.o0, o1 = T0.o1;
+      if (o1 - o0 <= 64) {
+        const int p = p0 + lane;
+        const bool owner = p < T0.p1;
+        const bool valid = o0 + lane < o1;
+        int mb = 0, me = 0;
+        if (owner) { mb = pt_start[p]; me = pt_start[p + 1]; }
+        double tv[3];
+        obs_term(cur, gcur, icur, valid, tv);
+        s_t[wv][0][lane] = tv[0]; s_t[wv][1][lane] = tv[1]; s_t[wv][2][lane] = tv[2];
+        wave_lds_sync();
+        if (owner) {
+          const Owner w = load_owner(p);
+          double T[3] = {0.0, 0.0, 0.0};
+          const int e = (MAVBA_BS_SKIP & 2) ? min(me, mb + 1) : me;
+          for (int i = mb; i < e; ++i) { T[0] += s_t[wv][0][i - o0]; T[1] += s_t[wv][1][i - o0]; T[2] += s_t[wv][2][i - o0]; }
+          owner_update(p, w, T, lane);
+        }
+        wave_lds_sync();
+        if (cost_partial) {
+          if (valid) cand_cost(cur, gcur.cam, (cur.pt - p0) & 63);
+          wave_lds_sync();
+        }
+      }
+      T0 = T1; T1 = T2; T2 = T3; cur = nxt; nxt = nn;
+#if MAVBA_BS_PREFETCH >= 1
+      gcur = gnxt;
+#endif
+#if MAVBA_BS_PREFETCH >= 2
+      icur = inxt;
+#endif
+    }
+  }
+  for (int k = t_first; k < num_long; k += S) {
+    const BacksubTile T0 = tiles[long_tiles[k]];
+    const int p = T0.p0, o0 = T0.o0, o1 = T0.o1;
+    const bool owner = lane == 0;
     double T[3] = {0.0, 0.0, 0.0};
-    for (int base = o0; base < o1; base += 256) {
-      const int o = base + tid;
-      const Obs q = base == o0 ? cur : load_obs(o);
-      double t[3];
-      obs_term(q, o < o1, t);
-      s_t[0][tid] = t[0]; s_t[1][tid] = t[1]; s_t[2][tid] = t[2];
-      __syncthreads();
+    for (int base = o0; base < o1; base += 64) {
+      const int o = base + lane;
+      const Obs q = load_obs(o);
+      double tv[3];
+      obs_term(q, gather_pt(q, o < o1), gather_im(q, o < o1), o < o1, tv);
+      s_t[wv][0][lane] = tv[0]; s_t[wv][1][lane] = tv[1]; s_t[wv][2][lane] = tv[2];
+      wave_lds_sync();
       if (owner) {
-        const int b = max(mb, base), e = (MAVBA_BS_SKIP & 2) ? min(me, max(mb, base) + 1) : min(me, base + 256);
-        for (int i = b; i < e; ++i) { T[0] += s_t[0][i - base]; T[1] += s_t[1][i - base]; T[2] += s_t[2][i - base]; }
-      }
-      __syncthreads();
-    }
-    if (owner) {
-      double d[3] = {0, 0, 0};
-      if (fr) {
-        const double q0 = -sp[0] * T[0], q1 = -sp[1] * T[1], q2 = -sp[2] * T[2];
-        const double z[3] = {q0 * G[0], q0 * G[1] + q1 * G[2], q0 * G[3] + q1 * G[4] + q2 * G[5]};
-        const double tt[3] = {hh[0] - z[0], hh[1] - z[1], hh[2] - z[2]};
-        double yp[3];
-        git_mul(G, tt, yp);
-#pragma unroll
-        for (int k = 0; k < 3; ++k) {
-          const double s = sp[k];
-          const double D2 = clampd(s * s * cu[k], dmin, dmax) / radius;
-          const double gs = s * gg[k];
-          a_model += 0.5 * yp[k] * (gs + D2 * yp[k]);
-          d[k] = -yp[k] * s;
-          a_step += d[k] * d[k];
+        const int e = (MAVBA_BS_SKIP & 2) ? (base == o0 ? 1 : 0) : min(o1 - base, 64);
+        for (int i = 0; i < e; ++i) { T[0] += s_t[wv][0][i]; T[1] += s_t[wv][1][i]; T[2] += s_t[wv][2][i]; }
+      }
+      wave_lds_sync();
+    }
+    if (owner) owner_update(p, load_owner(p), T, 0);
+    if (cost_partial) {
+      wave_lds_sync();
+      for (int base = o0; base < o1; base += 64) {
+        const int o = base + lane;
+        if (o < o1) {
+          const Obs c = load_obs(o);
+          cand_cost(c, img_cam[c.im], 0);
         }
       }
-#pragma unroll
-      for (int k = 0; k < 3; ++k) {
-        const double xn = Xo[k] + d[k];
-        cand_points[3 * (size_t)p + k] = xn;
-        delta_points[3 * (size_t)p + k] = d[k];
-        if (fr) a_x2 += xn * xn;
-        if (cost_partial) s_new[k][tid] = xn;
-      }
-    }
-    if (cost_partial) {
-      __syncthreads();
-      for (int base = o0; base < o1; base += 256) {
-        const int o = base + tid;
-        if (o < o1) {
-          const int pt = obs_pt[o], im = obs_img[o];
-          const double2 m = uv[o];
-          const int cam = img_cam[im];
-          double rec[9], kin[9], r[2];
-#pragma unroll
-          for (int k = 0; k < 9; ++k) rec[k] = cand_camrec[9 * im + k];
-#pragma unroll
-          for (int k = 0; k < 9; ++k) kin[k] = cand_intr[9 * cam + k];
-          const double Xn[3] = {s_new[0][pt - p0], s_new[1][pt - p0], s_new[2][pt - p0]};
-          obs_residual(cam_model[cam], rec, kin, Xn, m.x, m.y, r);
-          double w, half_rho;
-          cauchy_weight(r[0] * r[0] + r[1] * r[1], loss_b, loss_inv_b, w, half_rho);
-          if (pt_active && !pt_active[pt]) half_rho = 0.0;
-          a_cost += half_rho;
-        }
-      }
-      __syncthreads();
-    }
-    o0 = o0n; o1 = o1n; o0n = o0nn; o1n = o1nn; cur = nxt;
+      wave_lds_sync();
+    }
   }
   const double s0 = block_sum_256(a_step, s_red);
   const double s1 = block_sum_256(a_model, s_red);
@@ -1706,18 +1773,19 @@
   return gp < 1 ? 1 : gp;
 }
 void launch_backsub_points_jvp(hipStream_t st, int NP, int NPs, int NI, double radius, double dmin, double dmax,
-                               const SweepArgs& a, const int* pt_start, const double* delta_cam,
+                               const SweepArgs& a, const int* pt_start, const BacksubTile* tiles, int num_tiles,
+                               const int* long_tiles, int num_long, const double* img_step, const double* delta_cam,
                                const unsigned char* pt_free, const double* Gi, const double* h, const double* Cu,
                                const double* gu, const double* scale_pt, double* cand_points, double* delta_points,
                                double* partial, const double* cand_camrec, const double* cand_intr, double* cost_partial) {
   const int gp = backsub_points_grid(NP);
-  const double track = NP > 0 ? (double)a.N / NP : 1.0;
-  const int ppb = std::max(1, std::min(128, (int)(224.0 / std::max(track, 1.0))));
-  const int nblocks = (NP + ppb - 1) / ppb;
-  hipLaunchKernelGGL(k_backsub_points_packed, dim3(gp), dim3(256), 0, st, NP, NPs, NI, a.NC, a.N, ppb, nblocks, radius, dmin, dmax, a.loss_b,
-                     a.loss_inv_b, pt_start, a.obs_img, a.obs_pt, a.uv, a.img_cam, a.cam_model, a.camrec, a.intr, delta_cam, pt_free,
-                     Gi, h, Cu, gu, scale_pt, a.points, cand_points, delta_points, partial, cand_camrec, cand_intr, a.pt_active,
-                     cost_partial);
+  auto launch = [&](auto kernel) {
+    hipLaunchKernelGGL(kernel, dim3(gp), dim3(256), 0, st, NP, NPs, NI, a.NC, a.N, num_tiles, num_long, radius, dmin, dmax,
+                       a.loss_b, a.loss_inv_b, tiles, long_tiles, pt_start, a.obs_img, a.obs_pt, a.uv, a.img_cam, a.cam_model, a.camrec,
+                       a.intr, img_step, delta_cam, pt_free, Gi, h, Cu, gu, scale_pt, a.points, cand_points, delta_points, partial,
+                       cand_camrec, cand_intr, a.pt_active, cost_partial);
+  };
+  if (a.NC <= kBsCamsLds) launch(k_backsub_points<true>); else launch(k_backsub_points<false>);
 }
 
 int update_cameras_groups(int NI) { return std::max(1, (NI + kUpdImagesPerGroup - 1) / kUpdImagesPerGroup); }
@@ -1726,18 +1794,20 @@
     const double* __restrict__ scale_cam, const double* __restrict__ img_rec, const double* __restrict__ cam_rec,
     const double* __restrict__ poses, const double* __restrict__ intr, double* cand_poses,
     double* __restrict__ cand_intr, double* __restrict__ delta_cam, double* __restrict__ partial3,
-    double* __restrict__ cand_camrec) {
+    double* __restrict__ cand_camrec, const double* __restrict__ camrec, double* __restrict__ img_step) {
   __shared__ double s_red[4];
   update_cameras_body(blockIdx.x, NI, NC, cam_part, radius, dmin, dmax, y, scale_cam, img_rec, cam_rec, poses, intr, cand_poses, cand_intr,
-                      delta_cam, partial3, cand_camrec, s_red);
+                      delta_cam, partial3, cand_camrec, camrec, img_step, s_red);
 }
 void launch_update_cameras(hipStream_t st, int NI, int NC, bool cam_part, double radius, double dmin,
                            double dmax, const double* y, const double* scale_cam,
                            const double* img_rec, const double* cam_rec, const double* poses,
                            const double* intr, double* cand_poses, double* cand_intr,
-                           double* delta_cam, double* partial3, double* cand_camrec) {
+                           double* delta_cam, double* partial3, double* cand_camrec, const double* camrec,
+                           double* img_step) {
   hipLaunchKernelGGL(k_update_cameras, dim3(update_cameras_groups(NI)), dim3(256), 0, st, NI, NC, cam_part ? 1 : 0, radius, dmin,
-                     dmax, y, scale_cam, img_rec, cam_rec, poses, intr, cand_poses, cand_intr, delta_cam, partial3, cand_camrec);
+                     dmax, y, scale_cam, img_rec, cam_rec, poses, intr, cand_poses, cand_intr, delta_cam, partial3, cand_camrec,
+                     camrec, img_step);
 }
 
 __global__ void __launch_bounds__(256) k_reduce_cols(const double* __restrict__ partial, int rows, int cols,
diff --git a/mavmap_amd/csrc/lm_bodies.h b/mavmap_amd/csrc/lm_bodies.h
--- a/mavmap_amd/csrc/lm_bodies.h
+++ b/mavmap_amd/csrc/lm_bodies.h
@@ -144,7 +144,7 @@
                                                     const double* y, const double* scale_cam, const double* img_rec,
                                                     const double* cam_rec, const double* poses, const double* intr,
                                                     double* cand_poses, double* cand_intr, double* delta_cam, double* partial3,
-                                                    double* cand_camrec, double* s_red) {
+                                                    double* cand_camrec, const double* camrec, double* img_step, double* s_red) {
   const int i0 = vb * kUpdImagesPerGroup, i1 = min(i0 + kUpdImagesPerGroup, NI);
   double a_step = 0.0, a_model = 0.0, a_x2 = 0.0;
   auto one = [&](int t) {
@@ -176,13 +176,25 @@
   const double s1 = block_sum_256(a_model, s_red);
   const double s2 = block_sum_256(a_x2, s_red);
   if (threadIdx.x == 0) { partial3[3 * vb] = s0; partial3[3 * vb + 1] = s1; partial3[3 * vb + 2] = s2; }
-  if (cand_camrec) {
+  if (cand_camrec || img_step) {
     __syncthreads();
     for (int i = i0 + threadIdx.x; i < i1; i += 256) {
-      double rec[9];
-      cam_prepare(cand_poses + 6 * i, rec);
-#pragma unroll
-      for (int k = 0; k < 9; ++k) cand_camrec[9 * i + k] = rec[k];
+      if (cand_camrec) {
+        double rec[9];
+        cam_prepare(cand_poses + 6 * i, rec);
+#pragma unroll
+        for (int k = 0; k < 9; ++k) cand_camrec[9 * i + k] = rec[k];
+      }
+      if (img_step) {
+        double rec[9], dc[6], step[6];
+#pragma unroll
+        for (int k = 0; k < 9; ++k) rec[k] = camrec[9 * i + k];
+#pragma unroll
+        for (int k = 0; k < 6; ++k) dc[k] = delta_cam[6 * i + k];
+        image_step_record(rec, dc, step);
+#pragma unroll
+        for (int k = 0; k < 6; ++k) img_step[6 * i + k] = step[k];
+      }
     }
   }
 }
diff --git a/mavmap_amd/csrc/session.h b/mavmap_amd/csrc/session.h
--- a/mavmap_amd/csrc/session.h
+++ b/mavmap_amd/csrc/session.h
@@ -257,6 +257,10 @@
       d_cam_img_start, d_cam_imgs, d_prior_img, d_prior_start, d_q_pt, d_q_cam, d_q_start, d_pt_count;
   DevBuf<FrontTile> d_front_tiles;
   int num_front_tiles = 0;
+  DevBuf<BacksubTile> d_backsub_tiles;
+  int num_backsub_tiles = 0;
+  DevBuf<int> d_backsub_long;
+  int num_backsub_long = 0;
   DevBuf<FrontTile> d_tail_tiles;
   int num_tail_tiles = 0, tail_begin = 0;
   bool front_ok = false;
@@ -299,7 +303,7 @@
   DevBuf<double> d_sweep_partial, d_camsum , d_img_intr_tmp, d_cam_partial;
   DevBuf<double> d_prior_res, d_prior_jac, d_prior_cost;
   DevBuf<double> d_Epose, d_Eintr, d_Wk, d_part[3];
-  DevBuf<double> d_M, d_L, d_y, d_diag_ws, d_delta_cam, d_delta_pts, d_norm_partial, d_step_partial, d_scal;
+  DevBuf<double> d_M, d_L, d_y, d_diag_ws, d_delta_cam, d_img_step, d_delta_pts, d_norm_partial, d_step_partial, d_scal;
   DevBuf<double> d_rnorm, d_perr;
   DevBuf<int> d_pt_orig;
   DevBuf<int> d_perm32;
@@ -453,6 +457,7 @@
   }
   bool wait_publication(double* h);
   void build_front_tiles(const std::vector<int>& q_start);
+  void build_backsub_tiles_table();
   void build_tiles(const std::vector<int>& q_start, int first, DevBuf<FrontTile>& out, int& count);
   void ensure_planes();
   bool fused_now() const { return fused_ok && rows_ok; }
diff --git a/mavmap_amd/csrc/session_build.hip b/mavmap_amd/csrc/session_build.hip
--- a/mavmap_amd/csrc/session_build.hip
+++ b/mavmap_amd/csrc/session_build.hip
@@ -409,6 +409,7 @@
   d_Epose.alloc((size_t)std::max(N, 1) * kPoseRec);
   d_y.alloc(n_pad); d_y.zero(st);
   d_delta_cam.alloc(n_pad); d_delta_pts.alloc(nP * 3);
+  d_img_step.alloc((size_t)std::max(NI, 1) * 6);
   d_norm_partial.alloc((size_t)(512 + kStateNormsCamBlocks) * 2); d_step_partial.alloc((size_t)(1024 + update_cameras_groups(NI) + 2) * 3);
   d_scal.alloc(SC_COUNT); d_scal.zero(st);
   d_rnorm.alloc(std::max(N, 1)); d_perr.alloc(nP);
@@ -742,6 +743,7 @@
   d_Eintr.alloc((size_t)std::max(Q, 1) * kIntrRec);
   if (planes_ready) d_Wk.alloc((size_t)std::max(Q, 1) * 27);
   build_front_tiles(q_start);
+  build_backsub_tiles_table();
 
   lap("flags + intr entries");
   std::vector<unsigned char> pt_mode(NP, 0);
@@ -1351,6 +1353,30 @@
   lap("upload terms");
 }
 
+std::vector<BacksubTile> mavba::build_backsub_tiles(int NP, const int* pt_start) {
+  std::vector<BacksubTile> tiles;
+  int p0 = 0;
+  for (int p = 0; p < NP; ++p) {
+    const int c = pt_start[p + 1] - pt_start[p];
+    if (p > p0 && (pt_start[p] - pt_start[p0] + c > 64 || p - p0 >= 64)) {
+      tiles.push_back(BacksubTile{p0, p, pt_start[p0], pt_start[p]});
+      p0 = p;
+    }
+  }
+  if (NP > p0) tiles.push_back(BacksubTile{p0, NP, pt_start[p0], pt_start[NP]});
+  return tiles;
+}
+void mavba_session::build_backsub_tiles_table() {
+  const std::vector<BacksubTile> tiles = build_backsub_tiles(NP, h_pt_start.data());
+  num_backsub_tiles = (int)tiles.size();
+  d_backsub_tiles.upload(tiles, st);
+  std::vector<int> long_tiles;
+  for (int k = 0; k < num_backsub_tiles; ++k)
+    if (tiles[k].o1 - tiles[k].o0 > 64) long_tiles.push_back(k);
+  num_backsub_long = (int)long_tiles.size();
+  d_backsub_long.upload(long_tiles, st);
+}
+
 void mavba_session::build_front_tiles(const std::vector<int>& q_start) {
   const bool planes_only = std::getenv("MAVBA_FRONT_PLANES") != nullptr;
   front_ok = !planes_only;
diff --git a/mavmap_amd/csrc/session_lm.hip b/mavmap_amd/csrc/session_lm.hip
--- a/mavmap_amd/csrc/session_lm.hip
+++ b/mavmap_amd/csrc/session_lm.hip
@@ -242,6 +242,7 @@
     u.scale_cam = d_scale_cam.p; u.img_rec = d_img_rec; u.cam_rec = d_cam_rec; u.poses = d_poses.p; u.intr = d_intr.p;
     u.cand_poses = d_cposes.p; u.cand_intr = d_cintr.p; u.delta_cam = d_delta_cam.p;
     u.partial3 = d_step_partial.p + 3 * (size_t)backsub_points_grid(NP); u.cand_camrec = d_ccamrec.p;
+    u.camrec = d_camrec.p; u.img_step = d_img_step.p;
   }
   timed_split("chol_factor", "chol_backsolve", [&](hipEvent_t mid) {
     cameras_updated = dense_spd_solve_device(st, d_M.p, n_mat, d_ymat.p, d_scal.p + SC_FAIL, d_diag_ws.p, d_L.p, chol_struct, d_col_var.p, d_y.p,
@@ -276,14 +277,14 @@
     timed("update_cameras", [&] {
       launch_update_cameras(st, NI, NC, rank == 0, r, dmin, dmax, d_y.p, d_scale_cam.p, d_img_rec, d_cam_rec,
                             d_poses.p, d_intr.p, d_cposes.p, d_cintr.p, d_delta_cam.p, d_step_partial.p + 3 * (size_t)rows,
-                            d_ccamrec.p);
+                            d_ccamrec.p, d_camrec.p, d_img_step.p);
     });
   cameras_updated = false;
-  static const long long fuse_max_obs = [] { const char* e = std::getenv("MAVBA_COST_FUSE_MAX_OBS"); return e ? std::atoll(e) : 500000ll; }();
+  const long long fuse_max_obs = [] { const char* e = std::getenv("MAVBA_COST_FUSE_MAX_OBS"); return e ? std::atoll(e) : 3000000ll; }();
   const bool cost_separate = (long long)N > fuse_max_obs;
   timed("backsub_points", [&] {
     launch_backsub_points_jvp(st, NP, NPs, NI, r, dmin, dmax, sweep_args(d_camrec.p, d_intr.p, d_points.p), d_pt_start.p,
-                              d_delta_cam.p, d_pt_free.p, d_Gi.p, d_h.p, d_Cu.p, d_gu.p, d_scale_pt.p, d_cpoints.p,
+                              d_backsub_tiles.p, num_backsub_tiles, d_backsub_long.p, num_backsub_long, d_img_step.p, d_delta_cam.p, d_pt_free.p, d_Gi.p, d_h.p, d_Cu.p, d_gu.p, d_scale_pt.p, d_cpoints.p,
                               d_delta_pts.p, d_step_partial.p, d_ccamrec.p, d_cintr.p, cost_separate ? nullptr : d_sweep_partial.p);
   });
   SweepArgs a = sweep_args(d_ccamrec.p, d_cintr.p, d_cpoints.p);
```
